# PRBonn/LiDiff

Hardware: NVIDIA H100
Metric: denoising_steps_per_sec_180k_pts_T50 (higher is better)
Workload: dtype fp16x3 split tensor-core MMA, fp32 accumulate (fp32 CUDA cores for the Cin=3 stem), fp64 DPM update

## Files before the change

### include/lidiff_b200.h

```cpp
#ifndef LIDIFF_B200_H_
#define LIDIFF_B200_H_

#include <stdint.h>
#include <stddef.h>

#ifdef __cplusplus
extern "C" {
#endif

#define LB2_OK            0
#define LB2_ERR_ARG      -1
#define LB2_ERR_CUDA     -2
#define LB2_ERR_UNSUP    -3

#define LB2_KEY_EMPTY 0xFFFFFFFFFFFFFFFFull

int         lb2_create(int device, void** handle);
void        lb2_destroy(void* handle);
const char* lb2_last_error(void* handle);
int         lb2_version(void);
int64_t     lb2_launch_count(void* handle);
int         lb2_read_status(void* handle, void* stream);

typedef struct {
    uint64_t* keys;
    int32_t*  vals;
    int32_t   cap_table;
} lb2_grid;

int lb2_quantize(void* h, void* stream, const float* x, int64_t n_elem, float resolution, int div_mode,
                 float* out_coord);

size_t lb2_unique_scratch_bytes(int64_t n_cap);
int lb2_unique_build(void* h, void* stream,
                     const float* in_f, const int32_t* in_i, const int32_t* d_nin, int32_t n_cap,
                     int32_t ts_floor, lb2_grid grid,
                     int32_t* out_coords, int32_t* inverse, int32_t* d_nout, void* scratch);

size_t lb2_voxel_mean_scratch_bytes(int32_t m_cap, int32_t c);
int lb2_voxel_mean(void* h, void* stream, const float* feats, const int32_t* inverse, int32_t n,
                   int32_t c, const int32_t* d_m, int32_t m_cap, float* out, void* scratch);

int lb2_kernel_map(void* h, void* stream, lb2_grid grid_in, const int32_t* out_coords,
                   const int32_t* d_nout, int32_t nout_cap, int32_t ks, int32_t step,
                   int32_t* nbr, int64_t nbr_stride, uint64_t* pair_count, uint32_t* row_mask);

int lb2_kernel_map_self(void* h, void* stream, lb2_grid grid, const int32_t* coords, const int32_t* d_n, int32_t n_cap,
                        int32_t step, int32_t* nbr, int64_t nbr_stride, uint64_t* pair_count, uint32_t* row_mask);

size_t lb2_row_order_scratch_bytes(int32_t n_cap);
int lb2_row_order(void* h, void* stream, const uint32_t* row_mask, const int32_t* d_n, int32_t n_cap,
                  int32_t kvol, int32_t* perm, void* scratch, const int32_t* coords, int32_t coord_shift);

int lb2_tile_order(void* h, void* stream, const uint32_t* row_mask, const int32_t* row_perm, const int32_t* d_n, int32_t n_cap,
                   int32_t* order128, int32_t* order256, void* scratch);

typedef struct {
    const float*   in1;
    const float*   in2;
    const float*   residual;
    float*         out;
    const float*   gate_table;
    const int32_t* gate_idx;
    float*         out_gated;
    const float*   pre_add;
    const void*    in1_h;
    const void*    in2_h;
    void*          out_h;
    void*          out_gated_h;
    const void*    residual_h;
} lb2_conv_io;

typedef struct {
    int32_t        c1, c2, cout, kvol;
    const float*   weight;
    const void*    weight_packed;
    const float*   scale;
    const float*   shift;
    int32_t        relu;
    const int32_t* nbr;
    int64_t        nbr_stride;
    const int32_t* d_mout;
    int32_t        mout_cap;
    const int32_t* row_perm;
    const uint32_t* row_mask;
    int32_t        npass;
    lb2_conv_io    io[2];
    const int32_t* tile_order128;
    const int32_t* tile_order256;
} lb2_conv_desc;

#define LB2_ALGO_AUTO  0
#define LB2_ALGO_FFMA  1
#define LB2_ALGO_TC    2
#define LB2_ALGO_TC_TILE 3
int lb2_spconv_forward(void* h, void* stream, const lb2_conv_desc* d, int algo);

typedef struct {
    int32_t        c1, c2, cout, kvol;
    const void*    weight_packed;
    const int32_t* pair_in;
    const int32_t* pair_out;
    const int32_t* koff;
    const int32_t* tile_off;
    int32_t        npass;
    const float*   in1[2];
    const float*   in2[2];
    const void*    in1_h[2];
    const void*    in2_h[2];
    float*         out[2];
    const int32_t* d_zero_rows;
    int32_t        zero_rows_cap;
} lb2_scatter_desc;
size_t lb2_pair_list_scratch_bytes(void);
int lb2_pair_list(void* h, void* stream, const int32_t* nbr, int64_t nbr_stride, const int32_t* d_nout,
                  int32_t nout_cap, int32_t kvol, int32_t skip_k, int32_t* pair_in, int32_t* pair_out,
                  int32_t* koff, int32_t* tile_off, void* scratch);
int lb2_spconv_scatter_supported(int32_t c1, int32_t c2, int32_t cout, int32_t kvol);
int lb2_spconv_scatter(void* h, void* stream, const lb2_scatter_desc* d);

size_t lb2_packed_weight_bytes(int32_t kvol, int32_t cin, int32_t cout);
int lb2_pack_weights(void* h, void* stream, const float* weight, int32_t kvol, int32_t cin, int32_t cout,
                     void* packed);

int lb2_nn_match(void* h, void* stream, const int32_t* q_coords, const int32_t* d_nq, int32_t nq_cap,
                 const int32_t* k_coords, const int32_t* d_nk, int32_t nk_cap, int32_t batch_scale,
                 int32_t* idx);

int lb2_nn_match_grid(void* h, void* stream, const int32_t* q_coords, const int32_t* d_nq, int32_t nq_cap,
                      const int32_t* k_coords, const int32_t* d_nk, int32_t nk_cap, lb2_grid key_grid,
                      int32_t key_stride, int32_t max_ring, int32_t* idx);

size_t lb2_nn_table_bytes(void);
int lb2_nn_table_build(void* h, void* stream, const int32_t* k_coords, const int32_t* d_nk, int32_t nk_cap, void* table);
int lb2_nn_match_table(void* h, void* stream, const int32_t* q_coords, const int32_t* d_nq, int32_t nq_cap,
                       const int32_t* k_coords, const int32_t* d_nk, int32_t nk_cap, const void* table,
                       int32_t key_stride, int32_t max_ring, int32_t* idx);

size_t lb2_nn_tree_bytes(int32_t nk_cap);
int lb2_nn_tree_build(void* h, void* stream, const int32_t* k_coords, const int32_t* d_nk, int32_t nk_cap, void* tree);
int lb2_nn_match_tree(void* h, void* stream, const int32_t* q_coords, const int32_t* d_nq, int32_t nq_cap,
                      const void* tree, int32_t nk_cap, const int32_t* k_coords, const int32_t* hint_of,
                      const int32_t* hint_idx, int32_t* idx);

int lb2_linear(void* h, void* stream, const float* x, int64_t ldx, const float* w, const float* b,
               const float* addend, int64_t ld_addend, int32_t m_cap, const int32_t* d_m,
               int32_t n_in, int32_t n_out, int32_t act, float* y, int64_t ldy,
               const float* prebias, int32_t pre_act);

int lb2_head_mlp(void* h, void* stream, const float* x, int64_t ldx, int64_t x_pass_stride, const float* w0, const float* b0,
                 const float* w1, const float* b1, int32_t m_cap, const int32_t* d_m, int32_t n_in, int32_t n_hid,
                 int32_t n_out, int32_t out_act, int32_t npass, float* y, int64_t ldy, int64_t y_pass_stride);

int lb2_gate_mul(void* h, void* stream, const float* x, const float* table, const int32_t* idx,
                 const int32_t* d_m, int32_t m_cap, int32_t c, float* out, void* out_h);

int lb2_gather_rows(void* h, void* stream, const float* src, const int32_t* idx, int32_t n, int32_t c,
                    float* out);

typedef struct {
    double c_sample, c_x0, c_noise, sigma_s, alpha_s, inv_r0;
    float  guidance_w, resolution;
    int32_t second_order, div_mode, f64_state;
} lb2_dpm_coef;
int lb2_guidance_dpm_step(void* h, void* stream, const float* eps_c, const float* eps_u,
                          const int32_t* inverse, const float* x_t, const double* x_init,
                          const float* noise, double* x0_state, int64_t n_points, lb2_dpm_coef coef,
                          float* eps_out, float* x_next, float* coord_next ,
                          const float* batch_col );

int lb2_farthest_point_sample(void* h, void* stream, const double* pts, int32_t n, int32_t n_samples,
                              int32_t* out_idx, double* dist_scratch);

int64_t lb2_fps_batched_capacity(void* h);
int lb2_farthest_point_sample_batched(void* h, void* stream, const double* pts, const int64_t* d_offsets, int32_t n_scans,
                                      int32_t max_n, int32_t n_samples, int32_t* out_idx);


size_t lb2_pc_tree_bytes(int32_t n_cap);
size_t lb2_pc_nn_scratch_bytes(int32_t nq_cap);
int lb2_pc_tree_build(void* h, void* stream, const double* pts, int32_t n, void* tree);
int lb2_pc_nn(void* h, void* stream, const double* q, int32_t nq, const void* tree, double* dist, int32_t* idx, void* scratch);

int lb2_pc_knn(void* h, void* stream, const void* tree, int32_t n, int32_t k, int32_t* idx, double* d2);
int lb2_pc_normals(void* h, void* stream, const double* pts, int32_t n, const int32_t* idx, int32_t k, double* normals);

int lb2_voxel_occupancy(void* h, void* stream, const double* pts, int32_t n, const double* edges, int32_t bins,
                        uint32_t* bits, uint32_t* counts, uint64_t* n_in);

int lb2_occupancy_confusion(void* h, void* stream, const uint32_t* bits_gt, const uint32_t* bits_pred, int64_t nbits, uint64_t* out);

int lb2_occupancy_bev(void* h, void* stream, const uint32_t* bits, int32_t bins, uint32_t* bev);

size_t lb2_jsd_scratch_bytes(int64_t n);
int lb2_jsd(void* h, void* stream, const uint32_t* hist_a, const uint32_t* hist_b, int64_t n, double* out, void* scratch);

size_t lb2_dist_stats_scratch_bytes(int32_t nt);
int lb2_dist_stats(void* h, void* stream, const double* dist, int32_t n, const double* thresholds, int32_t nt,
                   double* sum_out, uint64_t* counts_out, void* scratch);

#define LB2_MAP_AXIS_BITS 21
typedef struct { float m[12]; } lb2_pose;

int lb2_map_rehash(void* h, void* stream, lb2_grid old_table, lb2_grid table);

size_t lb2_map_scan_scratch_bytes(int32_t n_cap);
int lb2_map_scan(void* h, void* stream, const float* points, const uint32_t* labels, int32_t n, lb2_pose pose, float voxel_size,
                 int32_t div_mode, lb2_grid table, float* map, int32_t map_n, int32_t map_cap, int32_t* d_out, void* scratch);

#ifdef __cplusplus
}
#endif
#endif
```

### lidiff_b200/_lib.py

```python
from __future__ import annotations

import ctypes as C
import os
import threading

import torch

_SO = os.path.join(os.path.dirname(os.path.abspath(__file__)), "_C", "liblidiff_b200.so")

ALGO_AUTO, ALGO_FFMA, ALGO_TC, ALGO_TC_TILE = 0, 1, 2, 3


class Grid(C.Structure):
    _fields_ = [("keys", C.c_void_p), ("vals", C.c_void_p), ("cap_table", C.c_int32)]


class ConvIO(C.Structure):
    _fields_ = [("in1", C.c_void_p), ("in2", C.c_void_p), ("residual", C.c_void_p), ("out", C.c_void_p),
                ("gate_table", C.c_void_p), ("gate_idx", C.c_void_p), ("out_gated", C.c_void_p), ("pre_add", C.c_void_p),
                ("in1_h", C.c_void_p), ("in2_h", C.c_void_p), ("out_h", C.c_void_p), ("out_gated_h", C.c_void_p),
                ("residual_h", C.c_void_p)]


class ConvDesc(C.Structure):
    _fields_ = [("c1", C.c_int32), ("c2", C.c_int32), ("cout", C.c_int32), ("kvol", C.c_int32),
                ("weight", C.c_void_p), ("weight_packed", C.c_void_p),
                ("scale", C.c_void_p), ("shift", C.c_void_p), ("relu", C.c_int32),
                ("nbr", C.c_void_p), ("nbr_stride", C.c_int64),
                ("d_mout", C.c_void_p), ("mout_cap", C.c_int32), ("row_perm", C.c_void_p), ("row_mask", C.c_void_p),
                ("npass", C.c_int32),
                ("io", ConvIO * 2),
                ("tile_order128", C.c_void_p), ("tile_order256", C.c_void_p)]


class ScatterDesc(C.Structure):
    _fields_ = [("c1", C.c_int32), ("c2", C.c_int32), ("cout", C.c_int32), ("kvol", C.c_int32),
                ("weight_packed", C.c_void_p), ("pair_in", C.c_void_p), ("pair_out", C.c_void_p),
                ("koff", C.c_void_p), ("tile_off", C.c_void_p), ("npass", C.c_int32),
                ("in1", C.c_void_p * 2), ("in2", C.c_void_p * 2), ("in1_h", C.c_void_p * 2), ("in2_h", C.c_void_p * 2),
                ("out", C.c_void_p * 2),
                ("d_zero_rows", C.c_void_p), ("zero_rows_cap", C.c_int32)]


class DpmCoef(C.Structure):
    _fields_ = [("c_sample", C.c_double), ("c_x0", C.c_double), ("c_noise", C.c_double),
                ("sigma_s", C.c_double), ("alpha_s", C.c_double), ("inv_r0", C.c_double),
                ("guidance_w", C.c_float), ("resolution", C.c_float),
                ("second_order", C.c_int32), ("div_mode", C.c_int32), ("f64_state", C.c_int32)]


EXPORTS = [
    "lb2_create", "lb2_destroy", "lb2_last_error", "lb2_version", "lb2_launch_count", "lb2_read_status",
    "lb2_tile_order",
    "lb2_quantize", "lb2_unique_scratch_bytes", "lb2_unique_build", "lb2_voxel_mean_scratch_bytes", "lb2_voxel_mean", "lb2_kernel_map",
    "lb2_spconv_forward", "lb2_packed_weight_bytes", "lb2_pack_weights", "lb2_nn_match", "lb2_linear",
    "lb2_gate_mul", "lb2_gather_rows", "lb2_head_mlp", "lb2_kernel_map_self", "lb2_guidance_dpm_step", "lb2_farthest_point_sample",
    "lb2_row_order", "lb2_row_order_scratch_bytes", "lb2_nn_match_grid",
    "lb2_nn_table_bytes", "lb2_nn_table_build", "lb2_nn_match_table",
    "lb2_nn_tree_bytes", "lb2_nn_tree_build", "lb2_nn_match_tree",
    "lb2_pair_list", "lb2_pair_list_scratch_bytes", "lb2_spconv_scatter", "lb2_spconv_scatter_supported",
    "lb2_pc_tree_bytes", "lb2_pc_nn_scratch_bytes", "lb2_pc_tree_build", "lb2_pc_nn", "lb2_voxel_occupancy", "lb2_occupancy_confusion",
    "lb2_occupancy_bev", "lb2_jsd_scratch_bytes", "lb2_jsd", "lb2_dist_stats_scratch_bytes", "lb2_dist_stats",
    "lb2_map_rehash", "lb2_map_scan_scratch_bytes", "lb2_map_scan",
    "lb2_pc_knn", "lb2_pc_normals", "lb2_fps_batched_capacity", "lb2_farthest_point_sample_batched",
]


class Pose(C.Structure):
    _fields_ = [("m", C.c_float * 12)]


def _ptr(t):
    if t is None:
        return None
    if isinstance(t, int):
        return t
    return t.data_ptr()


class Lib:

    def __init__(self, path: str = _SO):
        if not os.path.exists(path):
            raise RuntimeError(f"lidiff_b200: CUDA library not built ({path}); run `python -c 'import __graft_entry__ as g; g.build()'` "
                               "or lidiff_b200/csrc/build.sh — there is no CPU fallback")
        self.path = path
        self.dll = C.CDLL(path)
        d = self.dll
        d.lb2_create.argtypes = [C.c_int, C.POINTER(C.c_void_p)]
        d.lb2_destroy.argtypes = [C.c_void_p]
        d.lb2_destroy.restype = None
        d.lb2_last_error.argtypes = [C.c_void_p]
        d.lb2_last_error.restype = C.c_char_p
        d.lb2_launch_count.argtypes = [C.c_void_p]
        d.lb2_launch_count.restype = C.c_int64
        d.lb2_read_status.argtypes = [C.c_void_p, C.c_void_p]
        d.lb2_unique_scratch_bytes.argtypes = [C.c_int64]
        d.lb2_unique_scratch_bytes.restype = C.c_size_t
        d.lb2_voxel_mean_scratch_bytes.argtypes = [C.c_int32, C.c_int32]
        d.lb2_voxel_mean_scratch_bytes.restype = C.c_size_t
        d.lb2_packed_weight_bytes.argtypes = [C.c_int32] * 3
        d.lb2_packed_weight_bytes.restype = C.c_size_t
        vp, i32, i64, f32 = C.c_void_p, C.c_int32, C.c_int64, C.c_float
        d.lb2_quantize.argtypes = [vp, vp, vp, i64, f32, C.c_int, vp]
        d.lb2_unique_build.argtypes = [vp, vp, vp, vp, vp, i32, i32, Grid, vp, vp, vp, vp]
        d.lb2_voxel_mean.argtypes = [vp, vp, vp, vp, i32, i32, vp, i32, vp, vp]
        d.lb2_kernel_map.argtypes = [vp, vp, Grid, vp, vp, i32, i32, i32, vp, i64, vp, vp]
        d.lb2_kernel_map_self.argtypes = [vp, vp, Grid, vp, vp, i32, i32, vp, i64, vp, vp]
        d.lb2_row_order.argtypes = [vp, vp, vp, vp, i32, i32, vp, vp, vp, i32]
        d.lb2_tile_order.argtypes = [vp, vp, vp, vp, vp, i32, vp, vp, vp]
        d.lb2_row_order_scratch_bytes.restype = C.c_size_t
        d.lb2_row_order_scratch_bytes.argtypes = [i32]
        d.lb2_spconv_forward.argtypes = [vp, vp, C.POINTER(ConvDesc), C.c_int]
        d.lb2_pack_weights.argtypes = [vp, vp, vp, i32, i32, i32, vp]
        d.lb2_nn_match.argtypes = [vp, vp, vp, vp, i32, vp, vp, i32, i32, vp]
        d.lb2_pair_list.argtypes = [vp, vp, vp, i64, vp, i32, i32, i32, vp, vp, vp, vp, vp]
        d.lb2_pair_list_scratch_bytes.restype = C.c_size_t
        d.lb2_spconv_scatter.argtypes = [vp, vp, C.POINTER(ScatterDesc)]
        d.lb2_spconv_scatter_supported.argtypes = [i32, i32, i32, i32]
        d.lb2_nn_table_bytes.restype = C.c_size_t
        d.lb2_nn_tree_bytes.restype = C.c_size_t
        d.lb2_nn_tree_bytes.argtypes = [i32]
        d.lb2_nn_tree_build.argtypes = [vp, vp, vp, vp, i32, vp]
        d.lb2_nn_match_tree.argtypes = [vp, vp, vp, vp, i32, vp, i32, vp, vp, vp, vp]
        d.lb2_nn_table_build.argtypes = [vp, vp, vp, vp, i32, vp]
        d.lb2_nn_match_table.argtypes = [vp, vp, vp, vp, i32, vp, vp, i32, vp, i32, i32, vp]
        d.lb2_nn_match_grid.argtypes = [vp, vp, vp, vp, i32, vp, vp, i32, Grid, i32, i32, vp]
        d.lb2_linear.argtypes = [vp, vp, vp, i64, vp, vp, vp, i64, i32, vp, i32, i32, i32, vp, i64,
                                 vp, i32]
        d.lb2_gate_mul.argtypes = [vp, vp, vp, vp, vp, vp, i32, i32, vp, vp]
        d.lb2_gather_rows.argtypes = [vp, vp, vp, vp, i32, i32, vp]
        d.lb2_head_mlp.argtypes = [vp, vp, vp, i64, i64, vp, vp, vp, vp, i32, vp, i32, i32, i32, i32, i32, vp, i64, i64]
        d.lb2_guidance_dpm_step.argtypes = [vp, vp, vp, vp, vp, vp, vp, vp, vp, i64, DpmCoef, vp, vp, vp, vp]
        d.lb2_farthest_point_sample.argtypes = [vp, vp, vp, i32, i32, vp, vp]
        d.lb2_fps_batched_capacity.argtypes = [vp]
        d.lb2_fps_batched_capacity.restype = C.c_int64
        d.lb2_farthest_point_sample_batched.argtypes = [vp, vp, vp, vp, i32, i32, i32, vp]
        for f, a in (("lb2_pc_tree_bytes", i32), ("lb2_pc_nn_scratch_bytes", i32), ("lb2_jsd_scratch_bytes", i64),
                     ("lb2_dist_stats_scratch_bytes", i32)):
            getattr(d, f).argtypes = [a]
            getattr(d, f).restype = C.c_size_t
        d.lb2_pc_tree_build.argtypes = [vp, vp, vp, i32, vp]
        d.lb2_pc_nn.argtypes = [vp, vp, vp, i32, vp, vp, vp, vp]
        d.lb2_pc_knn.argtypes = [vp, vp, vp, i32, i32, vp, vp]
        d.lb2_pc_normals.argtypes = [vp, vp, vp, i32, vp, i32, vp]
        d.lb2_voxel_occupancy.argtypes = [vp, vp, vp, i32, vp, i32, vp, vp, vp]
        d.lb2_occupancy_confusion.argtypes = [vp, vp, vp, vp, i64, vp]
        d.lb2_occupancy_bev.argtypes = [vp, vp, vp, i32, vp]
        d.lb2_jsd.argtypes = [vp, vp, vp, vp, i64, vp, vp]
        d.lb2_dist_stats.argtypes = [vp, vp, vp, i32, vp, i32, vp, vp, vp]
        d.lb2_map_rehash.argtypes = [vp, vp, Grid, Grid]
        d.lb2_map_scan_scratch_bytes.argtypes = [i32]
        d.lb2_map_scan_scratch_bytes.restype = C.c_size_t
        d.lb2_map_scan.argtypes = [vp, vp, vp, vp, i32, Pose, f32, i32, Grid, vp, i32, i32, vp, vp]
        self._handles = {}
        self._lock = threading.Lock()

    def missing_symbols(self):
        return [s for s in EXPORTS if not hasattr(self.dll, s)]

    def handle(self, device) -> "Handle":
        dev = torch.device(device)
        if dev.type != "cuda":
            raise RuntimeError("lidiff_b200 runs on CUDA (H100, sm_90a) only; no CPU fallback")
        idx = dev.index if dev.index is not None else torch.cuda.current_device()
        with self._lock:
            if idx not in self._handles:
                hp = C.c_void_p()
                rc = self.dll.lb2_create(idx, C.byref(hp))
                if rc != 0:
                    raise RuntimeError(f"lb2_create(device={idx}) failed with {rc} (needs an sm_90 GPU)")
                self._handles[idx] = Handle(self, hp, idx)
            return self._handles[idx]


class Handle:
    def __init__(self, lib: Lib, hp, device_index: int):
        self.lib, self.dll, self.hp, self.device_index = lib, lib.dll, hp, device_index
        self.device = torch.device("cuda", device_index)

    def _stream(self):
        return torch.cuda.current_stream(self.device).cuda_stream

    def _check(self, rc, what):
        if rc != 0:
            msg = self.dll.lb2_last_error(self.hp)
            raise RuntimeError(f"{what} failed ({rc}): {msg.decode() if msg else ''}")

    def launch_count(self) -> int:
        return int(self.dll.lb2_launch_count(self.hp))

    def read_status(self) -> int:
        return int(self.dll.lb2_read_status(self.hp, self._stream()))

    def new_grid(self, n_cap: int):
        cap = 1 << max(4, (2 * n_cap - 1).bit_length())
        keys = torch.empty(cap, dtype=torch.int64, device=self.device)
        vals = torch.empty(2 * cap, dtype=torch.int32, device=self.device)
        return (keys, vals, cap)

    @staticmethod
    def _grid(g):
        return Grid(g[0].data_ptr(), g[1].data_ptr(), g[2])

    def unique_scratch(self, n_cap: int) -> torch.Tensor:
        nbytes = int(self.dll.lb2_unique_scratch_bytes(n_cap))
        return torch.empty(nbytes, dtype=torch.uint8, device=self.device)

    def quantize(self, x, resolution, div_mode, out):
        self._check(self.dll.lb2_quantize(self.hp, self._stream(), _ptr(x), x.numel(), float(resolution), int(div_mode), _ptr(out)), "lb2_quantize")

    def unique_build(self, in_f, in_i, d_nin, n_cap, ts_floor, grid, out_coords, inverse, d_nout, scratch):
        self._check(self.dll.lb2_unique_build(self.hp, self._stream(), _ptr(in_f), _ptr(in_i), _ptr(d_nin), int(n_cap), int(ts_floor),
                                              self._grid(grid), _ptr(out_coords), _ptr(inverse), _ptr(d_nout), _ptr(scratch)), "lb2_unique_build")

    def voxel_mean_scratch(self, m_cap: int, c: int) -> torch.Tensor:
        nbytes = int(self.dll.lb2_voxel_mean_scratch_bytes(int(m_cap), int(c)))
        return torch.empty(nbytes, dtype=torch.uint8, device=self.device)

    def voxel_mean(self, feats, inverse, n, c, d_m, m_cap, out, scratch):
        self._check(self.dll.lb2_voxel_mean(self.hp, self._stream(), _ptr(feats), _ptr(inverse), int(n), int(c), _ptr(d_m), int(m_cap),
                                            _ptr(out), _ptr(scratch)), "lb2_voxel_mean")

    def kernel_map(self, grid_in, out_coords, d_nout, nout_cap, ks, step, nbr, nbr_stride, pair_count=None, row_mask=None):
        self._check(self.dll.lb2_kernel_map(self.hp, self._stream(), self._grid(grid_in), _ptr(out_coords), _ptr(d_nout), int(nout_cap),
                                            int(ks), int(step), _ptr(nbr), int(nbr_stride), _ptr(pair_count), _ptr(row_mask)), "lb2_kernel_map")

    def kernel_map_self(self, grid, coords, d_n, n_cap, step, nbr, nbr_stride, pair_count=None, row_mask=None):
        self._check(self.dll.lb2_kernel_map_self(self.hp, self._stream(), self._grid(grid), _ptr(coords), _ptr(d_n), int(n_cap), int(step),
                                                 _ptr(nbr), int(nbr_stride), _ptr(pair_count), _ptr(row_mask)), "lb2_kernel_map_self")

    def row_order_scratch_bytes(self, n_cap) -> int:
        return int(self.dll.lb2_row_order_scratch_bytes(int(n_cap)))

    def row_order(self, row_mask, d_n, n_cap, kvol, perm, scratch, coords=None, coord_shift=0):
        self._check(self.dll.lb2_row_order(self.hp, self._stream(), _ptr(row_mask), _ptr(d_n), int(n_cap), int(kvol), _ptr(perm), _ptr(scratch),
                                           _ptr(coords), int(coord_shift)), "lb2_row_order")

    def tile_order(self, row_mask, row_perm, d_n, n_cap, order128, order256, scratch):
        self._check(self.dll.lb2_tile_order(self.hp, self._stream(), _ptr(row_mask), _ptr(row_perm), _ptr(d_n), int(n_cap), _ptr(order128),
                                            _ptr(order256), _ptr(scratch)), "lb2_tile_order")

    def spconv(self, desc: ConvDesc, algo: int = ALGO_AUTO):
        self._check(self.dll.lb2_spconv_forward(self.hp, self._stream(), C.byref(desc), int(algo)), "lb2_spconv_forward")

    def pair_list(self, nbr, nbr_stride, d_nout, nout_cap, kvol, skip_k, pair_in, pair_out, koff, tile_off, scratch):
        self._check(self.dll.lb2_pair_list(self.hp, self._stream(), _ptr(nbr), int(nbr_stride), _ptr(d_nout), int(nout_cap), int(kvol), int(skip_k),
                                           _ptr(pair_in), _ptr(pair_out), _ptr(koff), _ptr(tile_off), _ptr(scratch)), "lb2_pair_list")

    def scatter_supported(self, c1, c2, cout, kvol) -> bool:
        return bool(self.dll.lb2_spconv_scatter_supported(int(c1), int(c2), int(cout), int(kvol)))

    def spconv_scatter(self, desc: "ScatterDesc"):
        self._check(self.dll.lb2_spconv_scatter(self.hp, self._stream(), C.byref(desc)), "lb2_spconv_scatter")

    def packed_weight_bytes(self, kvol, cin, cout) -> int:
        return int(self.dll.lb2_packed_weight_bytes(kvol, cin, cout))

    def pack_weights(self, w: torch.Tensor):
        kvol, cin, cout = w.shape
        nbytes = self.packed_weight_bytes(kvol, cin, cout)
        if nbytes == 0:
            return None
        out = torch.empty(nbytes, dtype=torch.uint8, device=self.device)
        self._check(self.dll.lb2_pack_weights(self.hp, self._stream(), _ptr(w), kvol, cin, cout, _ptr(out)), "lb2_pack_weights")
        return out

    def nn_match(self, q, d_nq, nq_cap, k, d_nk, nk_cap, batch_scale, idx):
        self._check(self.dll.lb2_nn_match(self.hp, self._stream(), _ptr(q), _ptr(d_nq), int(nq_cap), _ptr(k), _ptr(d_nk), int(nk_cap),
                                          int(batch_scale), _ptr(idx)), "lb2_nn_match")

    def nn_match_grid(self, q, d_nq, nq_cap, k, d_nk, nk_cap, key_grid, key_stride, max_ring, idx):
        self._check(self.dll.lb2_nn_match_grid(self.hp, self._stream(), _ptr(q), _ptr(d_nq), int(nq_cap), _ptr(k), _ptr(d_nk), int(nk_cap),
                                               self._grid(key_grid), int(key_stride), int(max_ring), _ptr(idx)), "lb2_nn_match_grid")

    def nn_table(self, k, d_nk, nk_cap):
        t = torch.empty(int(self.dll.lb2_nn_table_bytes()), dtype=torch.uint8, device=self.device)
        self._check(self.dll.lb2_nn_table_build(self.hp, self._stream(), _ptr(k), _ptr(d_nk), int(nk_cap), _ptr(t)), "lb2_nn_table_build")
        return t

    def nn_tree(self, k, d_nk, nk_cap, out=None):
        nbytes = int(self.dll.lb2_nn_tree_bytes(int(nk_cap)))
        t = out if (out is not None and out.numel() == nbytes) else torch.empty(nbytes, dtype=torch.uint8, device=self.device)
        self._check(self.dll.lb2_nn_tree_build(self.hp, self._stream(), _ptr(k), _ptr(d_nk), int(nk_cap), _ptr(t)), "lb2_nn_tree_build")
        return t

    def nn_match_tree(self, q, d_nq, nq_cap, tree, nk_cap, idx, k=None, hint_of=None, hint_idx=None):
        self._check(self.dll.lb2_nn_match_tree(self.hp, self._stream(), _ptr(q), _ptr(d_nq), int(nq_cap), _ptr(tree), int(nk_cap),
                                               _ptr(k), _ptr(hint_of), _ptr(hint_idx), _ptr(idx)), "lb2_nn_match_tree")

    def nn_match_table(self, q, d_nq, nq_cap, k, d_nk, nk_cap, table, key_stride, max_ring, idx):
        self._check(self.dll.lb2_nn_match_table(self.hp, self._stream(), _ptr(q), _ptr(d_nq), int(nq_cap), _ptr(k), _ptr(d_nk), int(nk_cap),
                                                _ptr(table), int(key_stride), int(max_ring), _ptr(idx)), "lb2_nn_match_table")

    def linear(self, x, ldx, w, b, addend, ld_add, m_cap, d_m, n_in, n_out, act, y, ldy, prebias=None, pre_act=0):
        self._check(self.dll.lb2_linear(self.hp, self._stream(), _ptr(x), int(ldx), _ptr(w), _ptr(b), _ptr(addend), int(ld_add), int(m_cap),
                                        _ptr(d_m), int(n_in), int(n_out), int(act), _ptr(y), int(ldy), _ptr(prebias), int(pre_act)), "lb2_linear")

    def head_mlp(self, x, ldx, x_pass_stride, w0, b0, w1, b1, m_cap, d_m, n_in, n_hid, n_out, out_act, npass, y, ldy, y_pass_stride):
        self._check(self.dll.lb2_head_mlp(self.hp, self._stream(), _ptr(x), int(ldx), int(x_pass_stride), _ptr(w0), _ptr(b0), _ptr(w1), _ptr(b1),
                                          int(m_cap), _ptr(d_m), int(n_in), int(n_hid), int(n_out), int(out_act), int(npass), _ptr(y), int(ldy),
                                          int(y_pass_stride)), "lb2_head_mlp")

    def gate_mul(self, x, table, idx, d_m, m_cap, c, out, out_h=None):
        self._check(self.dll.lb2_gate_mul(self.hp, self._stream(), _ptr(x), _ptr(table), _ptr(idx), _ptr(d_m), int(m_cap), int(c), _ptr(out),
                                          _ptr(out_h)), "lb2_gate_mul")

    def gather_rows(self, src, idx, n, c, out):
        self._check(self.dll.lb2_gather_rows(self.hp, self._stream(), _ptr(src), _ptr(idx), int(n), int(c), _ptr(out)), "lb2_gather_rows")

    def guidance_dpm_step(self, eps_c, eps_u, inverse, x_t, x_init, noise, x0_state, n_points, coef: DpmCoef,
                          eps_out, x_next, coord_next, batch_col=None):
        self._check(self.dll.lb2_guidance_dpm_step(self.hp, self._stream(), _ptr(eps_c), _ptr(eps_u), _ptr(inverse), _ptr(x_t), _ptr(x_init),
                                                   _ptr(noise), _ptr(x0_state), int(n_points), coef, _ptr(eps_out), _ptr(x_next),
                                                   _ptr(coord_next), _ptr(batch_col)), "lb2_guidance_dpm_step")

    def farthest_point_sample(self, pts, n, n_samples, out_idx, dist):
        self._check(self.dll.lb2_farthest_point_sample(self.hp, self._stream(), _ptr(pts), int(n), int(n_samples), _ptr(out_idx), _ptr(dist)),
                    "lb2_farthest_point_sample")

    def fps_batched_capacity(self) -> int:
        return int(self.dll.lb2_fps_batched_capacity(self.hp))

    def farthest_point_sample_batched(self, pts, offsets, n_scans, max_n, n_samples, out_idx):
        self._check(self.dll.lb2_farthest_point_sample_batched(self.hp, self._stream(), _ptr(pts), _ptr(offsets), int(n_scans), int(max_n),
                                                               int(n_samples), _ptr(out_idx)), "lb2_farthest_point_sample_batched")

    def _bytes(self, nbytes):
        return torch.empty(max(int(nbytes), 1), dtype=torch.uint8, device=self.device)

    def pc_tree(self, pts):
        n = pts.shape[0]
        tree = self._bytes(self.dll.lb2_pc_tree_bytes(n))
        self._check(self.dll.lb2_pc_tree_build(self.hp, self._stream(), _ptr(pts), int(n), _ptr(tree)), "lb2_pc_tree_build")
        return tree

    def pc_nn(self, q, tree, dist, idx=None):
        nq = q.shape[0]
        scratch = self._bytes(self.dll.lb2_pc_nn_scratch_bytes(nq))
        self._check(self.dll.lb2_pc_nn(self.hp, self._stream(), _ptr(q), int(nq), _ptr(tree), _ptr(dist), _ptr(idx), _ptr(scratch)),
                    "lb2_pc_nn")

    def pc_knn(self, tree, n, k, idx, d2=None):
        self._check(self.dll.lb2_pc_knn(self.hp, self._stream(), _ptr(tree), int(n), int(k), _ptr(idx), _ptr(d2)), "lb2_pc_knn")

    def pc_normals(self, pts, idx, normals):
        n, k = idx.shape
        self._check(self.dll.lb2_pc_normals(self.hp, self._stream(), _ptr(pts), int(n), _ptr(idx), int(k), _ptr(normals)), "lb2_pc_normals")

    def voxel_occupancy(self, pts, edges, bits=None, counts=None, n_in=None):
        bins = edges.shape[0] - 1
        self._check(self.dll.lb2_voxel_occupancy(self.hp, self._stream(), _ptr(pts), int(pts.shape[0]), _ptr(edges), int(bins), _ptr(bits),
                                                 _ptr(counts), _ptr(n_in)), "lb2_voxel_occupancy")

    def occupancy_confusion(self, bits_gt, bits_pred, nbits, out):
        self._check(self.dll.lb2_occupancy_confusion(self.hp, self._stream(), _ptr(bits_gt), _ptr(bits_pred), int(nbits), _ptr(out)),
                    "lb2_occupancy_confusion")

    def occupancy_bev(self, bits, bins, bev):
        self._check(self.dll.lb2_occupancy_bev(self.hp, self._stream(), _ptr(bits), int(bins), _ptr(bev)), "lb2_occupancy_bev")

    def jsd(self, hist_a, hist_b, out):
        n = hist_a.numel()
        scratch = self._bytes(self.dll.lb2_jsd_scratch_bytes(n))
        self._check(self.dll.lb2_jsd(self.hp, self._stream(), _ptr(hist_a), _ptr(hist_b), int(n), _ptr(out), _ptr(scratch)), "lb2_jsd")

    def dist_stats(self, dist, thresholds, sum_out, counts_out):
        nt = thresholds.shape[0]
        scratch = self._bytes(self.dll.lb2_dist_stats_scratch_bytes(nt))
        self._check(self.dll.lb2_dist_stats(self.hp, self._stream(), _ptr(dist), int(dist.shape[0]), _ptr(thresholds), int(nt), _ptr(sum_out),
                                            _ptr(counts_out), _ptr(scratch)), "lb2_dist_stats")

    def new_map_table(self, cap: int):
        return (torch.empty(cap, dtype=torch.int64, device=self.device), torch.empty(2 * cap, dtype=torch.int32, device=self.device), cap)

    def map_rehash(self, old, table):
        self._check(self.dll.lb2_map_rehash(self.hp, self._stream(), self._grid(old) if old is not None else Grid(None, None, 0),
                                            self._grid(table)), "lb2_map_rehash")

    def map_scan_scratch(self, n_cap: int) -> torch.Tensor:
        return self._bytes(self.dll.lb2_map_scan_scratch_bytes(int(n_cap)))

    def map_scan(self, points, labels, pose12, voxel_size, div_mode, table, map_buf, map_n, out, scratch):
        pose = Pose((C.c_float * 12)(*[float(v) for v in pose12]))
        self._check(self.dll.lb2_map_scan(self.hp, self._stream(), _ptr(points), _ptr(labels), int(points.shape[0]), pose, float(voxel_size),
                                          int(div_mode), self._grid(table), _ptr(map_buf), int(map_n), int(map_buf.shape[0]), _ptr(out),
                                          _ptr(scratch)), "lb2_map_scan")


_LIB = None


def get_lib() -> Lib:
    global _LIB
    if _LIB is None:
        _LIB = Lib()
    return _LIB


def get_handle(device) -> Handle:
    return get_lib().handle(device)
```

### lidiff_b200/csrc/api.cu

```cuda
#include "common.cuh"

int lb2_spconv_ffma_launch(Lb2Handle* h, cudaStream_t s, const lb2_conv_desc* d);
int lb2_spconv_tc_launch(Lb2Handle* h, cudaStream_t s, const lb2_conv_desc* d);
bool lb2_spconv_tc_supported(const lb2_conv_desc* d);

extern "C" int lb2_spconv_forward(void* handle, void* stream, const lb2_conv_desc* d, int algo) {
    Lb2Handle* h = (Lb2Handle*)handle;
    LB2_REQUIRE(h, h && d, "spconv_forward null");
    LB2_REQUIRE(h, d->npass == 1 || d->npass == 2, "npass must be 1 or 2");
    LB2_REQUIRE(h, d->c1 > 0 && d->c2 >= 0 && d->cout > 0 && d->kvol > 0 && d->mout_cap > 0, "shape");
    LB2_REQUIRE(h, d->weight != nullptr, "weight");
    LB2_REQUIRE(h, (d->scale == nullptr) == (d->shift == nullptr), "scale/shift must come together");
    LB2_REQUIRE(h, d->nbr != nullptr || d->kvol == 1, "identity map only for kvol == 1");
    LB2_REQUIRE(h, d->nbr == nullptr || d->nbr_stride >= d->mout_cap, "nbr_stride");
    bool have_f32 = true;
    for (int p = 0; p < d->npass; ++p) {
        const lb2_conv_io& io = d->io[p];
        const bool f = io.in1 && (d->c2 == 0 || io.in2), hh = io.in1_h && (d->c2 == 0 || io.in2_h);
        LB2_REQUIRE(h, f || hh, "in1 / in2 (fp32 tensors or their split companions)");
        LB2_REQUIRE(h, d->c2 > 0 || (io.in2 == nullptr && io.in2_h == nullptr), "in2 / c2 mismatch");
        LB2_REQUIRE(h, !hh || (d->c1 % 8 == 0 && d->c2 % 8 == 0), "split companions need channel counts that are multiples of 8");
        LB2_REQUIRE(h, io.out || io.out_gated || io.out_h || io.out_gated_h, "no output");
        have_f32 = have_f32 && f;
    }
    LB2_REQUIRE(h, d->c2 == 0 || d->c1 % 16 == 0, "c1 must be a multiple of 16 when in2 is given");
    cudaStream_t s = (cudaStream_t)stream;
    if (algo == LB2_ALGO_TC || algo == LB2_ALGO_TC_TILE) {
        if (!d->weight_packed || !lb2_spconv_tc_supported(d))
            return lb2_fail(h, LB2_ERR_UNSUP, "tensor-core variant does not support this layer%s", "");
        return lb2_spconv_tc_launch(h, s, d);
    }
    if (algo == LB2_ALGO_AUTO && d->weight_packed && lb2_spconv_tc_supported(d)) return lb2_spconv_tc_launch(h, s, d);
    if (!have_f32) return lb2_fail(h, LB2_ERR_UNSUP, "companion-only inputs need a tensor-core variant that takes this layer%s", "");
    return lb2_spconv_ffma_launch(h, s, d);
}
```

### lidiff_b200/csrc/coords.cu

```cuda
#include "common.cuh"
#include <stdlib.h>
#include <limits.h>
#include <algorithm>

extern "C" int lb2_version(void) { return 100; }

extern "C" int lb2_create(int device, void** handle) {
    if (!handle) return LB2_ERR_ARG;
    *handle = nullptr;
    int n = 0;
    if (cudaGetDeviceCount(&n) != cudaSuccess || n <= 0 || device < 0 || device >= n) return LB2_ERR_CUDA;
    if (cudaSetDevice(device) != cudaSuccess) return LB2_ERR_CUDA;
    cudaDeviceProp prop;
    if (cudaGetDeviceProperties(&prop, device) != cudaSuccess) return LB2_ERR_CUDA;
    if (prop.major != 9) return LB2_ERR_UNSUP;
    Lb2Handle* h = new Lb2Handle();
    h->device = device; h->num_sms = prop.multiProcessorCount; h->launches = 0; h->err[0] = 0; h->configured = 0;
    if (cudaMalloc(&h->d_status, sizeof(int32_t)) != cudaSuccess) { delete h; return LB2_ERR_CUDA; }
    cudaMemset(h->d_status, 0, sizeof(int32_t));
    *handle = h;
    return LB2_OK;
}

extern "C" void lb2_destroy(void* handle) {
    Lb2Handle* h = (Lb2Handle*)handle;
    if (!h) return;
    cudaFree(h->d_status);
    delete h;
}

extern "C" const char* lb2_last_error(void* handle) {
    return handle ? ((Lb2Handle*)handle)->err : "null handle";
}

extern "C" int64_t lb2_launch_count(void* handle) { return handle ? ((Lb2Handle*)handle)->launches : -1; }

extern "C" int lb2_read_status(void* handle, void* stream) {
    Lb2Handle* h = (Lb2Handle*)handle;
    if (!h) return LB2_ERR_ARG;
    int32_t v = 0;
    cudaStream_t s = (cudaStream_t)stream;
    if (cudaMemcpyAsync(&v, h->d_status, sizeof(v), cudaMemcpyDeviceToHost, s) != cudaSuccess) return LB2_ERR_CUDA;
    if (cudaMemsetAsync(h->d_status, 0, sizeof(v), s) != cudaSuccess) return LB2_ERR_CUDA;
    if (cudaStreamSynchronize(s) != cudaSuccess) return LB2_ERR_CUDA;
    return v;
}

__global__ void k_quantize(const float* __restrict__ x, long long n, float res, float inv_res, int div_mode,
                           float* __restrict__ out) {
    long long i = (long long)blockIdx.x * blockDim.x + threadIdx.x;
    if (i >= n) return;
    float v = x[i];
    float q = div_mode == 0 ? __fdiv_rn(v, res) : __fmul_rn(v, inv_res);
    out[i] = rintf(q);
}

extern "C" int lb2_quantize(void* handle, void* stream, const float* x, int64_t n_elem, float resolution,
                            int div_mode, float* out_coord) {
    Lb2Handle* h = (Lb2Handle*)handle;
    LB2_REQUIRE(h, h && x && out_coord && resolution > 0.f, "quantize");
    if (n_elem == 0) return LB2_OK;
    float inv = 1.0f / resolution;
    k_quantize<<<cdiv(n_elem, 256), 256, 0, (cudaStream_t)stream>>>(x, n_elem, resolution, inv, div_mode, out_coord);
    LB2_POST_LAUNCH(h, "k_quantize");
    return LB2_OK;
}

#define SCAN_THREADS 512
#define SCAN_ITEMS   4
#define SCAN_TILE    (SCAN_THREADS * SCAN_ITEMS)

struct UniqueScratch {
    int* slot_of;
    int* rank;
    int* bsum;
};

extern "C" size_t lb2_unique_scratch_bytes(int64_t n_cap) {
    size_t a = ((size_t)n_cap * sizeof(int) + 255) / 256 * 256;
    return 2 * a + SCAN_TILE * sizeof(int) + 256;
}

static UniqueScratch carve(void* scratch, int64_t n_cap) {
    size_t a = ((size_t)n_cap * sizeof(int) + 255) / 256 * 256;
    char* p = (char*)scratch;
    UniqueScratch s;
    s.slot_of = (int*)p; s.rank = (int*)(p + a); s.bsum = (int*)(p + 2 * a);
    return s;
}

__global__ void k_grid_clear(unsigned long long* keys, int* vals, int cap) {
    int i = blockIdx.x * blockDim.x + threadIdx.x;
    if (i < cap) { keys[i] = LB2_KEY_EMPTY; vals[i] = INT_MAX; vals[cap + i] = -1; }
}

__device__ __forceinline__ int4 load_row(const float* __restrict__ in_f, const int* __restrict__ in_i, int i, int ts, bool* nan = nullptr) {
    int4 c;
    if (in_f) {
        float4 f = __ldg(reinterpret_cast<const float4*>(in_f) + i);
        c = make_int4((int)floorf(f.x), (int)floorf(f.y), (int)floorf(f.z), (int)floorf(f.w));
        if (nan) *nan = isnan(f.x) || isnan(f.y) || isnan(f.z) || isnan(f.w);
    } else {
        c = __ldg(reinterpret_cast<const int4*>(in_i) + i);
    }
    if (ts > 0) { c.y = floor_to_multiple(c.y, ts); c.z = floor_to_multiple(c.z, ts); c.w = floor_to_multiple(c.w, ts); }
    return c;
}

__global__ void k_grid_insert(const float* __restrict__ in_f, const int* __restrict__ in_i,
                              const int* __restrict__ d_n, int n_cap, int ts,
                              unsigned long long* keys, int* vals, unsigned mask,
                              int* __restrict__ slot_of, int* status) {
    int i = blockIdx.x * blockDim.x + threadIdx.x;
    int n = d_n ? min(*d_n, n_cap) : n_cap;
    if (i >= n) return;
    bool nan = false;
    int4 c = load_row(in_f, in_i, i, ts, &nan);
    unsigned long long key;
    if (!lb2_pack_key(c.x, c.y, c.z, c.w, key) || nan) atomicOr(status, 1);
    unsigned slot = lb2_hash(key) & mask;
    while (true) {
        unsigned long long prev = atomicCAS(keys + slot, (unsigned long long)LB2_KEY_EMPTY, key);
        if (prev == LB2_KEY_EMPTY || prev == key) break;
        slot = (slot + 1) & mask;
    }
    atomicMin(vals + slot, i);
    slot_of[i] = (int)slot;
}

__global__ void __launch_bounds__(SCAN_THREADS) k_scan_local(const int* __restrict__ slot_of, const int* __restrict__ vals,
                                                             const int* __restrict__ d_n, int n_cap,
                                                             int* __restrict__ rank, int* __restrict__ bsum) {
    __shared__ int warp_tot[SCAN_THREADS / 32];
    int n = d_n ? min(*d_n, n_cap) : n_cap;
    int base = blockIdx.x * SCAN_TILE + threadIdx.x * SCAN_ITEMS;
    int f[SCAN_ITEMS], tsum = 0;
#pragma unroll
    for (int j = 0; j < SCAN_ITEMS; ++j) {
        int i = base + j;
        f[j] = (i < n) ? (vals[slot_of[i]] == i) : 0;
        tsum += f[j];
    }
    int lane = threadIdx.x & 31, w = threadIdx.x >> 5;
    int incl = tsum;
#pragma unroll
    for (int d = 1; d < 32; d <<= 1) { int v = __shfl_up_sync(0xffffffffu, incl, d); if (lane >= d) incl += v; }
    if (lane == 31) warp_tot[w] = incl;
    __syncthreads();
    if (w == 0) {
        int v = (lane < SCAN_THREADS / 32) ? warp_tot[lane] : 0, inc2 = v;
#pragma unroll
        for (int d = 1; d < 32; d <<= 1) { int u = __shfl_up_sync(0xffffffffu, inc2, d); if (lane >= d) inc2 += u; }
        if (lane < SCAN_THREADS / 32) warp_tot[lane] = inc2 - v;
        if (lane == SCAN_THREADS / 32 - 1) bsum[blockIdx.x] = inc2;
    }
    __syncthreads();
    int excl = warp_tot[w] + incl - tsum;
#pragma unroll
    for (int j = 0; j < SCAN_ITEMS; ++j) {
        int i = base + j;
        if (i < n) rank[i] = f[j] ? excl : -1;
        excl += f[j];
    }
}

__global__ void __launch_bounds__(SCAN_THREADS) k_scan_bsum(int* __restrict__ bsum, int nblocks, int* __restrict__ d_total) {
    __shared__ int warp_tot[SCAN_THREADS / 32];
    int base = threadIdx.x * SCAN_ITEMS;
    int v[SCAN_ITEMS], tsum = 0;
#pragma unroll
    for (int j = 0; j < SCAN_ITEMS; ++j) { v[j] = (base + j < nblocks) ? bsum[base + j] : 0; tsum += v[j]; }
    int lane = threadIdx.x & 31, w = threadIdx.x >> 5;
    int incl = tsum;
#pragma unroll
    for (int d = 1; d < 32; d <<= 1) { int u = __shfl_up_sync(0xffffffffu, incl, d); if (lane >= d) incl += u; }
    if (lane == 31) warp_tot[w] = incl;
    __syncthreads();
    if (w == 0) {
        int x = (lane < SCAN_THREADS / 32) ? warp_tot[lane] : 0, inc2 = x;
#pragma unroll
        for (int d = 1; d < 32; d <<= 1) { int u = __shfl_up_sync(0xffffffffu, inc2, d); if (lane >= d) inc2 += u; }
        if (lane < SCAN_THREADS / 32) warp_tot[lane] = inc2 - x;
        if (lane == SCAN_THREADS / 32 - 1) *d_total = inc2;
    }
    __syncthreads();
    int excl = warp_tot[w] + incl - tsum;
#pragma unroll
    for (int j = 0; j < SCAN_ITEMS; ++j) { if (base + j < nblocks) bsum[base + j] = excl; excl += v[j]; }
}

__global__ void k_unique_emit(const float* __restrict__ in_f, const int* __restrict__ in_i,
                              const int* __restrict__ d_n, int n_cap, int ts,
                              const int* __restrict__ slot_of, const int* __restrict__ rank,
                              const int* __restrict__ bsum, int* __restrict__ vals, int cap,
                              int4* __restrict__ out_coords) {
    int i = blockIdx.x * blockDim.x + threadIdx.x;
    int n = d_n ? min(*d_n, n_cap) : n_cap;
    if (i >= n) return;
    int r = rank[i];
    if (r < 0) return;
    r += bsum[i / SCAN_TILE];
    vals[cap + slot_of[i]] = r;
    out_coords[r] = load_row(in_f, in_i, i, ts);
}

__global__ void k_unique_inverse(const int* __restrict__ d_n, int n_cap, const int* __restrict__ slot_of,
                                 const int* __restrict__ vals, int cap, int* __restrict__ inverse) {
    int i = blockIdx.x * blockDim.x + threadIdx.x;
    int n = d_n ? min(*d_n, n_cap) : n_cap;
    if (i < n) inverse[i] = vals[cap + slot_of[i]];
}

extern "C" int lb2_unique_build(void* handle, void* stream, const float* in_f, const int32_t* in_i,
                                const int32_t* d_nin, int32_t n_cap, int32_t ts_floor, lb2_grid grid,
                                int32_t* out_coords, int32_t* inverse, int32_t* d_nout, void* scratch) {
    Lb2Handle* h = (Lb2Handle*)handle;
    LB2_REQUIRE(h, h != nullptr, "handle");
    LB2_REQUIRE(h, (in_f != nullptr) != (in_i != nullptr), "exactly one of in_f / in_i");
    LB2_REQUIRE(h, grid.keys && grid.vals && out_coords && d_nout && scratch, "null buffer");
    LB2_REQUIRE(h, n_cap > 0 && n_cap <= SCAN_TILE * SCAN_TILE, "n_cap out of range (max 4M rows)");
    LB2_REQUIRE(h, grid.cap_table >= 2 && (grid.cap_table & (grid.cap_table - 1)) == 0, "cap_table must be a power of two");
    LB2_REQUIRE(h, (long long)grid.cap_table >= 2LL * n_cap, "cap_table must be >= 2 * n_cap");
    LB2_REQUIRE(h, ts_floor >= 0, "ts_floor");
    cudaStream_t s = (cudaStream_t)stream;
    UniqueScratch sc = carve(scratch, n_cap);
    unsigned long long* keys = (unsigned long long*)grid.keys;
    int cap = grid.cap_table;
    unsigned mask = (unsigned)cap - 1u;
    int nblk = (int)cdiv(n_cap, SCAN_TILE);

    k_grid_clear<<<cdiv(cap, 256), 256, 0, s>>>(keys, grid.vals, cap);
    LB2_POST_LAUNCH(h, "k_grid_clear");
    k_grid_insert<<<cdiv(n_cap, 256), 256, 0, s>>>(in_f, in_i, d_nin, n_cap, ts_floor, keys, grid.vals, mask, sc.slot_of, h->d_status);
    LB2_POST_LAUNCH(h, "k_grid_insert");
    k_scan_local<<<nblk, SCAN_THREADS, 0, s>>>(sc.slot_of, grid.vals, d_nin, n_cap, sc.rank, sc.bsum);
    LB2_POST_LAUNCH(h, "k_scan_local");
    k_scan_bsum<<<1, SCAN_THREADS, 0, s>>>(sc.bsum, nblk, d_nout);
    LB2_POST_LAUNCH(h, "k_scan_bsum");
    k_unique_emit<<<cdiv(n_cap, 256), 256, 0, s>>>(in_f, in_i, d_nin, n_cap, ts_floor, sc.slot_of, sc.rank, sc.bsum,
                                                  grid.vals, cap, (int4*)out_coords);
    LB2_POST_LAUNCH(h, "k_unique_emit");
    if (inverse) {
        k_unique_inverse<<<cdiv(n_cap, 256), 256, 0, s>>>(d_nin, n_cap, sc.slot_of, grid.vals, cap, inverse);
        LB2_POST_LAUNCH(h, "k_unique_inverse");
    }
    return LB2_OK;
}

__device__ __forceinline__ int voxel_fix_shift(float maxabs, int count) {
    int e;
    frexpf(maxabs, &e);
    return 61 - e - (32 - __clz(count));
}

__global__ void k_voxel_absmax(const float* __restrict__ feats, const int* __restrict__ inverse, int n, int c,
                               unsigned* __restrict__ maxabs, int* __restrict__ counts) {
    long long t = (long long)blockIdx.x * blockDim.x + threadIdx.x;
    if (t >= (long long)n * c) return;
    int i = (int)(t / c), j = (int)(t % c);
    int r = inverse[i];
    atomicMax(maxabs + (long long)r * c + j, __float_as_uint(fabsf(feats[t])));
    if (j == 0) atomicAdd(counts + r, 1);
}

__global__ void k_voxel_accum(const float* __restrict__ feats, const int* __restrict__ inverse, int n, int c,
                              const float* __restrict__ maxabs, const int* __restrict__ counts, unsigned long long* __restrict__ sums) {
    long long t = (long long)blockIdx.x * blockDim.x + threadIdx.x;
    if (t >= (long long)n * c) return;
    int i = (int)(t / c), j = (int)(t % c);
    int r = inverse[i];
    const long long e = (long long)r * c + j;
    const float m = maxabs[e];
    if (!(m > 0.f) || !isfinite(m)) return;
    const long long q = llrint(ldexp((double)feats[t], voxel_fix_shift(m, counts[r])));
    atomicAdd(sums + e, (unsigned long long)q);
}

__global__ void k_voxel_div(float* __restrict__ out, const int* __restrict__ counts, const unsigned long long* __restrict__ sums,
                            const int* __restrict__ d_m, int m_cap, int c) {
    long long t = (long long)blockIdx.x * blockDim.x + threadIdx.x;
    int m = d_m ? min(*d_m, m_cap) : m_cap;
    if (t >= (long long)m * c) return;
    const float mx = out[t];
    const int cnt = counts[t / c];
    if (!isfinite(mx)) { out[t] = __int_as_float(0x7fffffff); return; }
    if (!(mx > 0.f) || cnt == 0) { out[t] = cnt == 0 ? __fdiv_rn(0.f, 0.f) : 0.f; return; }
    const double sum = ldexp((double)(long long)sums[t], -voxel_fix_shift(mx, cnt));
    out[t] = __double2float_rn(sum / (double)cnt);
}

extern "C" size_t lb2_voxel_mean_scratch_bytes(int32_t m_cap, int32_t c) {
    return (size_t)m_cap * c * sizeof(unsigned long long) + (size_t)m_cap * sizeof(int);
}

extern "C" int lb2_voxel_mean(void* handle, void* stream, const float* feats, const int32_t* inverse, int32_t n,
                              int32_t c, const int32_t* d_m, int32_t m_cap, float* out, void* scratch) {
    Lb2Handle* h = (Lb2Handle*)handle;
    LB2_REQUIRE(h, h && feats && inverse && out && scratch && n > 0 && c > 0 && m_cap > 0, "voxel_mean");
    cudaStream_t s = (cudaStream_t)stream;
    unsigned long long* sums = (unsigned long long*)scratch;
    int* counts = (int*)(sums + (size_t)m_cap * c);
    if (cudaMemsetAsync(out, 0, (size_t)m_cap * c * sizeof(float), s) != cudaSuccess ||
        cudaMemsetAsync(scratch, 0, lb2_voxel_mean_scratch_bytes(m_cap, c), s) != cudaSuccess)
        return lb2_fail(h, LB2_ERR_CUDA, "voxel_mean memset%s", "");
    k_voxel_absmax<<<cdiv((long long)n * c, 256), 256, 0, s>>>(feats, inverse, n, c, (unsigned*)out, counts);
    LB2_POST_LAUNCH(h, "k_voxel_absmax");
    k_voxel_accum<<<cdiv((long long)n * c, 256), 256, 0, s>>>(feats, inverse, n, c, out, counts, sums);
    LB2_POST_LAUNCH(h, "k_voxel_accum");
    k_voxel_div<<<cdiv((long long)m_cap * c, 256), 256, 0, s>>>(out, counts, sums, d_m, m_cap, c);
    LB2_POST_LAUNCH(h, "k_voxel_div");
    return LB2_OK;
}

template <int KS>
__global__ void __launch_bounds__(128) k_kernel_map(const unsigned long long* __restrict__ keys, const int* __restrict__ rows, unsigned mask,
                                                    const int4* __restrict__ out_coords, const int* __restrict__ d_n, int n_cap,
                                                    int step, int* __restrict__ nbr, long long nbr_stride,
                                                    unsigned long long* __restrict__ pair_count, unsigned* __restrict__ row_mask) {
    constexpr int KV = KS * KS * KS;
    const int o = blockIdx.x * blockDim.x + threadIdx.x;
    const int n = d_n ? min(*d_n, n_cap) : n_cap;
    unsigned found = 0;
    if (o < n) {
        const int4 c = __ldg(out_coords + o);
        constexpr int cen = (KS & 1) ? KS / 2 : 0;
        int res[KV];
        unsigned long long key[KV], got[KV];
        unsigned slot[KV];
#pragma unroll
        for (int k = 0; k < KV; ++k) {
            const int kx = k % KS, ky = (k / KS) % KS, kz = k / (KS * KS);
            const int x = c.y + (kx - cen) * step, y = c.z + (ky - cen) * step, z = c.w + (kz - cen) * step;
            const bool ok = lb2_pack_key(c.x, x, y, z, key[k]);
            slot[k] = ok ? (lb2_hash(key[k]) & mask) : 0u;
            got[k] = ok ? __ldg(keys + slot[k]) : LB2_KEY_EMPTY;
            if (!ok) key[k] = ~LB2_KEY_EMPTY;
        }
#pragma unroll
        for (int k = 0; k < KV; ++k) {
            if (got[k] == key[k]) res[k] = __ldg(rows + slot[k]);
            else if (got[k] == LB2_KEY_EMPTY) res[k] = -1;
            else {
                unsigned sl = (slot[k] + 1) & mask;
                res[k] = -1;
                while (true) {
                    const unsigned long long kk = __ldg(keys + sl);
                    if (kk == key[k]) { res[k] = __ldg(rows + sl); break; }
                    if (kk == LB2_KEY_EMPTY) break;
                    sl = (sl + 1) & mask;
                }
            }
        }
#pragma unroll
        for (int k = 0; k < KV; ++k) {
            nbr[(long long)k * nbr_stride + o] = res[k];
            if (res[k] >= 0) found |= 1u << k;
        }
    } else if (o < n_cap) {
#pragma unroll
        for (int k = 0; k < KV; ++k) nbr[(long long)k * nbr_stride + o] = -1;
    }
    if (row_mask && o < n_cap) row_mask[o] = found;
    if (pair_count) {
        int cnt = __popc(found);
#pragma unroll
        for (int d = 16; d > 0; d >>= 1) cnt += __shfl_xor_sync(0xffffffffu, cnt, d);
        if ((threadIdx.x & 31) == 0 && cnt) atomicAdd(pair_count, (unsigned long long)cnt);
    }
}

extern "C" int lb2_kernel_map(void* handle, void* stream, lb2_grid grid_in, const int32_t* out_coords,
                              const int32_t* d_nout, int32_t nout_cap, int32_t ks, int32_t step,
                              int32_t* nbr, int64_t nbr_stride, uint64_t* pair_count, uint32_t* row_mask) {
    Lb2Handle* h = (Lb2Handle*)handle;
    LB2_REQUIRE(h, h && grid_in.keys && grid_in.vals && out_coords && nbr, "kernel_map null");
    LB2_REQUIRE(h, ks >= 1 && ks <= 3 && step != 0 && nout_cap > 0 && nbr_stride >= nout_cap, "kernel_map args");
    const unsigned long long* gk = (const unsigned long long*)grid_in.keys;
    const int* gr = grid_in.vals + grid_in.cap_table;
    const unsigned gm = (unsigned)grid_in.cap_table - 1u;
    const unsigned blocks = cdiv(nout_cap, 128);
    cudaStream_t s = (cudaStream_t)stream;
    if (ks == 3) k_kernel_map<3><<<blocks, 128, 0, s>>>(gk, gr, gm, (const int4*)out_coords, d_nout, nout_cap, step, nbr, nbr_stride, (unsigned long long*)pair_count, row_mask);
    else if (ks == 2) k_kernel_map<2><<<blocks, 128, 0, s>>>(gk, gr, gm, (const int4*)out_coords, d_nout, nout_cap, step, nbr, nbr_stride, (unsigned long long*)pair_count, row_mask);
    else k_kernel_map<1><<<blocks, 128, 0, s>>>(gk, gr, gm, (const int4*)out_coords, d_nout, nout_cap, step, nbr, nbr_stride, (unsigned long long*)pair_count, row_mask);
    LB2_POST_LAUNCH(h, "k_kernel_map");
    return LB2_OK;
}

__global__ void __launch_bounds__(128) k_kernel_map_self(const unsigned long long* __restrict__ keys, const int* __restrict__ rows, unsigned mask,
                                                         const int4* __restrict__ coords, const int* __restrict__ d_n, int n_cap, int step,
                                                         int* __restrict__ nbr, long long nbr_stride,
                                                         unsigned long long* __restrict__ pair_count, unsigned* __restrict__ row_mask) {
    constexpr int HALF = 13;
    const int o = blockIdx.x * blockDim.x + threadIdx.x;
    const int n = d_n ? min(*d_n, n_cap) : n_cap;
    unsigned found = 0;
    if (o < n) {
        const int4 c = __ldg(coords + o);
        int res[HALF];
        unsigned long long key[HALF], got[HALF];
        unsigned slot[HALF];
#pragma unroll
        for (int k = 0; k < HALF; ++k) {
            const int kx = k % 3, ky = (k / 3) % 3, kz = k / 9;
            const int x = c.y + (kx - 1) * step, y = c.z + (ky - 1) * step, z = c.w + (kz - 1) * step;
            const bool ok = lb2_pack_key(c.x, x, y, z, key[k]);
            slot[k] = ok ? (lb2_hash(key[k]) & mask) : 0u;
            got[k] = ok ? __ldg(keys + slot[k]) : LB2_KEY_EMPTY;
            if (!ok) key[k] = ~LB2_KEY_EMPTY;
        }
#pragma unroll
        for (int k = 0; k < HALF; ++k) {
            if (got[k] == key[k]) res[k] = __ldg(rows + slot[k]);
            else if (got[k] == LB2_KEY_EMPTY) res[k] = -1;
            else {
                unsigned sl = (slot[k] + 1) & mask;
                res[k] = -1;
                while (true) {
                    const unsigned long long kk = __ldg(keys + sl);
                    if (kk == key[k]) { res[k] = __ldg(rows + sl); break; }
                    if (kk == LB2_KEY_EMPTY) break;
                    sl = (sl + 1) & mask;
                }
            }
        }
#pragma unroll
        for (int k = 0; k < HALF; ++k) {
            nbr[(long long)k * nbr_stride + o] = res[k];
            if (res[k] >= 0) {
                found |= 1u << k;
                nbr[(long long)(26 - k) * nbr_stride + res[k]] = o;
                if (row_mask) atomicOr(row_mask + res[k], 1u << (26 - k));
            }
        }
        nbr[(long long)HALF * nbr_stride + o] = o;
        if (row_mask) atomicOr(row_mask + o, found | (1u << HALF));
    } else if (o < n_cap) {
#pragma unroll
        for (int k = 0; k <= HALF; ++k) nbr[(long long)k * nbr_stride + o] = -1;
    }
    if (pair_count) {
        int cnt = (o < n) ? 2 * __popc(found) + 1 : 0;
#pragma unroll
        for (int d = 16; d > 0; d >>= 1) cnt += __shfl_xor_sync(0xffffffffu, cnt, d);
        if ((threadIdx.x & 31) == 0 && cnt) atomicAdd(pair_count, (unsigned long long)cnt);
    }
}

extern "C" int lb2_kernel_map_self(void* handle, void* stream, lb2_grid grid, const int32_t* coords, const int32_t* d_n, int32_t n_cap,
                                   int32_t step, int32_t* nbr, int64_t nbr_stride, uint64_t* pair_count, uint32_t* row_mask) {
    Lb2Handle* h = (Lb2Handle*)handle;
    LB2_REQUIRE(h, h && grid.keys && grid.vals && coords && nbr, "kernel_map_self null");
    LB2_REQUIRE(h, step > 0 && n_cap > 0 && nbr_stride >= n_cap, "kernel_map_self args");
    cudaStream_t s = (cudaStream_t)stream;
    cudaError_t e = cudaMemsetAsync(nbr + 14 * nbr_stride, 0xff, (size_t)13 * nbr_stride * sizeof(int32_t), s);
    if (e == cudaSuccess && row_mask) e = cudaMemsetAsync(row_mask, 0, (size_t)n_cap * sizeof(uint32_t), s);
    if (e != cudaSuccess) return lb2_fail(h, LB2_ERR_CUDA, "kernel_map_self memset: %s", cudaGetErrorString(e));
    k_kernel_map_self<<<cdiv(n_cap, 128), 128, 0, s>>>((const unsigned long long*)grid.keys, grid.vals + grid.cap_table, (unsigned)grid.cap_table - 1u,
                                                       (const int4*)coords, d_n, n_cap, step, nbr, nbr_stride, (unsigned long long*)pair_count, row_mask);
    LB2_POST_LAUNCH(h, "k_kernel_map_self");
    return LB2_OK;
}

#define RS_BITS 9
#define RS_BINS (1 << RS_BITS)
#define RS_CHUNK 2048
#define RS_WARPS 8

__device__ __forceinline__ unsigned ro_key27(unsigned mask) {
    const unsigned extras = mask & ~(1u << 13);
    const unsigned k26 = ((mask >> 14) << 13) | (mask & 0x1fffu);
    return ((__popc(extras) >= 2) ? (1u << 26) : 0u) | k26;
}

__device__ __forceinline__ unsigned ro_part9(unsigned v) {
    v &= 0x1ffu;
    v = (v | (v << 16)) & 0x030000ffu;
    v = (v | (v << 8)) & 0x0300f00fu;
    v = (v | (v << 4)) & 0x030c30c3u;
    v = (v | (v << 2)) & 0x09249249u;
    return v;
}
__device__ __forceinline__ unsigned ro_morton(const int4 c, int shift) {
    return ro_part9((unsigned)(c.y >> shift)) | (ro_part9((unsigned)(c.z >> shift)) << 1) | (ro_part9((unsigned)(c.w >> shift)) << 2);
}

struct RsSrc {
    const unsigned* keys;
    const unsigned* mask;
    const int4* coords;
    const int* vals;
    int mode, coord_shift;
};
__device__ __forceinline__ unsigned rs_key(const RsSrc& s, int i) {
    switch (s.mode) {
        case 0: return s.keys[i];
        case 1: return ro_key27(s.mask[i]);
        case 2: return ro_morton(s.coords[i], s.coord_shift);
        case 4: return s.mask[i] & 0xffu;
        default: return ro_key27(s.mask[s.vals[i]]);
    }
}

__global__ void __launch_bounds__(256) k_rs_hist(const RsSrc src, const int* __restrict__ d_n, int n_cap, int shift, int* __restrict__ hist,
                                                 int* __restrict__ total) {
    __shared__ int sh[RS_BINS];
    for (int i = threadIdx.x; i < RS_BINS; i += blockDim.x) sh[i] = 0;
    __syncthreads();
    const int n = d_n ? min(*d_n, n_cap) : n_cap;
    const int lo = blockIdx.x * RS_CHUNK, hi = min(lo + RS_CHUNK, n);
    for (int i = lo + threadIdx.x; i < hi; i += blockDim.x) atomicAdd(&sh[(rs_key(src, i) >> shift) & (RS_BINS - 1)], 1);
    __syncthreads();
    for (int i = threadIdx.x; i < RS_BINS; i += blockDim.x) {
        hist[blockIdx.x * RS_BINS + i] = sh[i];
        if (sh[i]) atomicAdd(total + i, sh[i]);
    }
}

__global__ void __launch_bounds__(32 * RS_WARPS) k_rs_scatter(const RsSrc src, const int* __restrict__ d_n, int n_cap,
                                                              int shift, const int* __restrict__ hist, const int* __restrict__ total,
                                                              unsigned* __restrict__ keys_out, int* __restrict__ vals_out) {
    const int* __restrict__ vals_in = src.vals;
    __shared__ int cnt[RS_WARPS][RS_BINS];
    __shared__ int first[RS_BINS];
    const int warp = threadIdx.x >> 5, lane = threadIdx.x & 31;
    for (int i = threadIdx.x; i < RS_WARPS * RS_BINS; i += blockDim.x) (&cnt[0][0])[i] = 0;
    {
        const int t = threadIdx.x;
        const int t0 = total[2 * t], t1 = total[2 * t + 1];
        first[t] = t0 + t1;
        __syncthreads();
        for (int d = 1; d < RS_BINS / 2; d <<= 1) {
            const int u = (t >= d) ? first[t - d] : 0;
            __syncthreads();
            first[t] += u;
            __syncthreads();
        }
        const int excl = first[t] - (t0 + t1);
        int p0 = 0, p1 = 0;
#pragma unroll 8
        for (int b = 0; b < (int)blockIdx.x; ++b) {
            const int2 v = *reinterpret_cast<const int2*>(hist + b * RS_BINS + 2 * t);
            p0 += v.x; p1 += v.y;
        }
        __syncthreads();
        first[2 * t] = excl + p0;
        first[2 * t + 1] = excl + t0 + p1;
    }
    __syncthreads();
    const int n = d_n ? min(*d_n, n_cap) : n_cap;
    const int w0 = blockIdx.x * RS_CHUNK + warp * (RS_CHUNK / RS_WARPS);
    for (int g = 0; g < RS_CHUNK / RS_WARPS / 32; ++g) {
        const int i = w0 + g * 32 + lane;
        if (i < n) atomicAdd(&cnt[warp][(rs_key(src, i) >> shift) & (RS_BINS - 1)], 1);
    }
    __syncthreads();
    for (int bin = threadIdx.x; bin < RS_BINS; bin += blockDim.x) {
        int run = first[bin];
        for (int w = 0; w < RS_WARPS; ++w) { const int v = cnt[w][bin]; cnt[w][bin] = run; run += v; }
    }
    __syncthreads();
    for (int g = 0; g < RS_CHUNK / RS_WARPS / 32; ++g) {
        const int i = w0 + g * 32 + lane;
        const bool ok = i < n;
        const unsigned active = __ballot_sync(0xffffffffu, ok);
        if (ok) {
            const unsigned key = rs_key(src, i);
            const int val = vals_in ? vals_in[i] : i;
            const int d = (key >> shift) & (RS_BINS - 1);
            const unsigned peers = __match_any_sync(active, d);
            const int rank = __popc(peers & ((1u << lane) - 1u));
            const int pos = cnt[warp][d] + rank;
            __syncwarp(active);
            if (rank == 0) cnt[warp][d] += __popc(peers);
            __syncwarp(active);
            if (keys_out) keys_out[pos] = key;
            vals_out[pos] = val;
        }
    }
}

static int rs_blocks(int n_cap) { return cdiv(n_cap, RS_CHUNK); }

extern "C" size_t lb2_row_order_scratch_bytes(int32_t n_cap) {
    return ((size_t)RS_BINS * (rs_blocks(n_cap) + 6) + 3 * (size_t)n_cap) * sizeof(int);
}

extern "C" int lb2_row_order(void* handle, void* stream, const uint32_t* row_mask, const int32_t* d_n, int32_t n_cap,
                             int32_t kvol, int32_t* perm, void* scratch, const int32_t* coords, int32_t coord_shift) {
    Lb2Handle* h = (Lb2Handle*)handle;
    LB2_REQUIRE(h, h && row_mask && perm && scratch && n_cap > 0 && (kvol == 27 || (kvol >= 1 && kvol <= 8)), "row_order");
    LB2_REQUIRE(h, coord_shift >= 0 && coord_shift < 24, "row_order coord_shift");
    cudaStream_t s = (cudaStream_t)stream;
    if (kvol == 27) {
        const int nblk = rs_blocks(n_cap);
        int* hist = (int*)scratch;
        int* total = hist + (size_t)RS_BINS * nblk;
        unsigned* keys_a = (unsigned*)(total + 6 * RS_BINS);
        if (cudaMemsetAsync(total, 0, 6 * RS_BINS * sizeof(int), s) != cudaSuccess) return lb2_fail(h, LB2_ERR_CUDA, "row_order memset%s", "");
        unsigned* keys_b = keys_a + n_cap;
        int* vals_a = (int*)(keys_b + n_cap);
        const int npass = coords ? 6 : 3;
        for (int pass = 0; pass < npass; ++pass) {
            const int mp = coords ? pass - 3 : pass;
            const bool to_perm = coords ? (pass & 1) : !(pass & 1);
            RsSrc src;
            src.mask = row_mask; src.coords = (const int4*)coords; src.coord_shift = coord_shift;
            src.keys = (pass & 1) ? keys_a : keys_b;
            src.vals = (pass == 0) ? nullptr : (to_perm ? vals_a : perm);
            src.mode = (pass == 0) ? (coords ? 2 : 1) : ((coords && pass == 3) ? 3 : 0);
            unsigned* kout = (pass == npass - 1 || (coords && pass == 2)) ? nullptr : ((pass & 1) ? keys_b : keys_a);
            int* vout = to_perm ? perm : vals_a;
            const int shift = (mp >= 0 ? mp : pass) * RS_BITS;
            k_rs_hist<<<nblk, 256, 0, s>>>(src, d_n, n_cap, shift, hist, total + pass * RS_BINS);
            LB2_POST_LAUNCH(h, "k_rs_hist");
            k_rs_scatter<<<nblk, 32 * RS_WARPS, 0, s>>>(src, d_n, n_cap, shift, hist, total + pass * RS_BINS, kout, vout);
            LB2_POST_LAUNCH(h, "k_rs_scatter");
        }
        return LB2_OK;
    }
    const int nblk = rs_blocks(n_cap);
    int* hist = (int*)scratch;
    int* total = hist + (size_t)RS_BINS * nblk;
    if (cudaMemsetAsync(total, 0, RS_BINS * sizeof(int), s) != cudaSuccess) return lb2_fail(h, LB2_ERR_CUDA, "row_order memset%s", "");
    RsSrc src;
    src.mask = row_mask; src.coords = nullptr; src.coord_shift = 0; src.keys = nullptr; src.vals = nullptr; src.mode = 4;
    k_rs_hist<<<nblk, 256, 0, s>>>(src, d_n, n_cap, 0, hist, total);
    LB2_POST_LAUNCH(h, "k_rs_hist");
    k_rs_scatter<<<nblk, 32 * RS_WARPS, 0, s>>>(src, d_n, n_cap, 0, hist, total, nullptr, perm);
    LB2_POST_LAUNCH(h, "k_rs_scatter");
    return LB2_OK;
}

size_t rs_sort_scratch_bytes(int n_cap, int nbits) {
    return ((size_t)RS_BINS * (rs_blocks(n_cap) + cdiv(nbits, RS_BITS)) + 4 * (size_t)n_cap) * sizeof(int);
}

int rs_sort_keys(Lb2Handle* h, cudaStream_t s, const unsigned* keys, const int* d_n, int n_cap, int nbits, int* order, void* scratch) {
    const int nblk = rs_blocks(n_cap), npass = (int)cdiv(nbits, RS_BITS);
    int* hist = (int*)scratch;
    int* total = hist + (size_t)RS_BINS * nblk;
    unsigned* keys_a = (unsigned*)(total + (size_t)npass * RS_BINS);
    unsigned* keys_b = keys_a + n_cap;
    int* vals_a = (int*)(keys_b + n_cap);
    int* vals_b = vals_a + n_cap;
    if (cudaMemsetAsync(total, 0, (size_t)npass * RS_BINS * sizeof(int), s) != cudaSuccess) return lb2_fail(h, LB2_ERR_CUDA, "rs_sort memset%s", "");
    const unsigned* kin = keys;
    const int* vin = nullptr;
    for (int pass = 0; pass < npass; ++pass) {
        const bool last = pass == npass - 1;
        unsigned* kout = last ? nullptr : ((pass & 1) ? keys_b : keys_a);
        int* vout = last ? order : ((pass & 1) ? vals_b : vals_a);
        RsSrc src;
        src.keys = kin; src.mask = nullptr; src.coords = nullptr; src.vals = vin; src.mode = 0; src.coord_shift = 0;
        k_rs_hist<<<nblk, 256, 0, s>>>(src, d_n, n_cap, pass * RS_BITS, hist, total + pass * RS_BINS);
        LB2_POST_LAUNCH(h, "k_rs_hist");
        k_rs_scatter<<<nblk, 32 * RS_WARPS, 0, s>>>(src, d_n, n_cap, pass * RS_BITS, hist, total + pass * RS_BINS, kout, vout);
        LB2_POST_LAUNCH(h, "k_rs_scatter");
        kin = kout; vin = vout;
    }
    return LB2_OK;
}

#define NT_LEAF 4
#define NT_HDR 16

static int nt_nleaf(int nk_cap) { int n = 1; while (n * NT_LEAF < nk_cap) n <<= 1; return n; }
static size_t nt_sort_ints(int nk_cap) { return (size_t)RS_BINS * (rs_blocks(nk_cap) + 3) + 4 * (size_t)nk_cap; }

extern "C" size_t lb2_nn_tree_bytes(int32_t nk_cap) {
    return (NT_HDR + (size_t)2 * nt_nleaf(nk_cap) * 8 + 5 * (size_t)nt_nleaf(nk_cap) * NT_LEAF + nt_sort_ints(nk_cap)) * sizeof(int) + 64;
}

__global__ void k_nt_init(int* __restrict__ hdr, int nleaf, int nk_cap) {
    if (threadIdx.x < 3) { hdr[threadIdx.x] = 0x7fffffff; hdr[3 + threadIdx.x] = (int)0x80000000; }
    if (threadIdx.x == 0) { hdr[6] = 0; hdr[7] = nleaf; hdr[8] = nk_cap; }
}

__global__ void k_nt_minmax(const int4* __restrict__ keys, const int* __restrict__ d_nk, int nk_cap, int* __restrict__ hdr) {
    const int nk = d_nk ? min(*d_nk, nk_cap) : nk_cap;
    int lo[3] = {0x7fffffff, 0x7fffffff, 0x7fffffff}, hi[3] = {(int)0x80000000, (int)0x80000000, (int)0x80000000};
    for (int i = blockIdx.x * blockDim.x + threadIdx.x; i < nk; i += gridDim.x * blockDim.x) {
        const int4 c = __ldg(keys + i);
        lo[0] = min(lo[0], c.y); lo[1] = min(lo[1], c.z); lo[2] = min(lo[2], c.w);
        hi[0] = max(hi[0], c.y); hi[1] = max(hi[1], c.z); hi[2] = max(hi[2], c.w);
    }
#pragma unroll
    for (int a = 0; a < 3; ++a) {
#pragma unroll
        for (int o = 16; o > 0; o >>= 1) { lo[a] = min(lo[a], __shfl_xor_sync(0xffffffffu, lo[a], o)); hi[a] = max(hi[a], __shfl_xor_sync(0xffffffffu, hi[a], o)); }
        if ((threadIdx.x & 31) == 0) { atomicMin(hdr + a, lo[a]); atomicMax(hdr + 3 + a, hi[a]); }
    }
}

__device__ __forceinline__ unsigned nt_spread9(unsigned v) {
    unsigned r = 0;
#pragma unroll
    for (int b = 0; b < 9; ++b) r |= ((v >> b) & 1u) << (3 * b);
    return r;
}

__global__ void k_nt_morton(const int4* __restrict__ keys, const int* __restrict__ d_nk, int nk_cap, const int* __restrict__ hdr,
                            unsigned* __restrict__ codes) {
    const int nk = d_nk ? min(*d_nk, nk_cap) : nk_cap;
    const int i = blockIdx.x * blockDim.x + threadIdx.x;
    if (i >= nk) return;
    long long ext = 0;
#pragma unroll
    for (int a = 0; a < 3; ++a) ext = max(ext, (long long)hdr[3 + a] - (long long)hdr[a]);
    int shift = 0;
    while ((ext >> shift) > 511) ++shift;
    const int4 c = __ldg(keys + i);
    const unsigned x = (unsigned)(((long long)c.y - hdr[0]) >> shift), y = (unsigned)(((long long)c.z - hdr[1]) >> shift),
                   z = (unsigned)(((long long)c.w - hdr[2]) >> shift);
    codes[i] = nt_spread9(x) | (nt_spread9(y) << 1) | (nt_spread9(z) << 2);
}

__global__ void k_nt_gather(const int4* __restrict__ keys, const int* __restrict__ d_nk, int nk_cap, const int* __restrict__ order,
                            int slots, int4* __restrict__ skeys, int* __restrict__ sbatch) {
    const int nk = d_nk ? min(*d_nk, nk_cap) : nk_cap;
    const int i = blockIdx.x * blockDim.x + threadIdx.x;
    if (i >= slots) return;
    if (i >= nk) { skeys[i] = make_int4(0, 0, 0, -1); sbatch[i] = 0; return; }
    const int j = order[i];
    const int4 c = __ldg(keys + j);
    skeys[i] = make_int4(c.y, c.z, c.w, j);
    sbatch[i] = c.x;
}

__global__ void k_nt_leaves(const int4* __restrict__ skeys, const int* __restrict__ sbatch, const int* __restrict__ d_nk, int nk_cap,
                            int nleaf, int* __restrict__ nodes) {
    const int nk = d_nk ? min(*d_nk, nk_cap) : nk_cap;
    const int l = blockIdx.x * blockDim.x + threadIdx.x;
    if (l >= nleaf) return;
    int v[8] = {0x7fffffff, 0x7fffffff, 0x7fffffff, (int)0x80000000, (int)0x80000000, (int)0x80000000, 0x7fffffff, (int)0x80000000};
    for (int t = 0; t < NT_LEAF; ++t) {
        const int i = l * NT_LEAF + t;
        if (i >= nk) break;
        const int4 c = skeys[i];
        const int b = sbatch[i];
        v[0] = min(v[0], c.x); v[1] = min(v[1], c.y); v[2] = min(v[2], c.z);
        v[3] = max(v[3], c.x); v[4] = max(v[4], c.y); v[5] = max(v[5], c.z);
        v[6] = min(v[6], b); v[7] = max(v[7], b);
    }
    int* n = nodes + (size_t)(nleaf + l) * 8;
#pragma unroll
    for (int a = 0; a < 8; ++a) n[a] = v[a];
}

__global__ void __launch_bounds__(1024) k_nt_internal(int nleaf, int* __restrict__ nodes) {
    for (int first = nleaf >> 1; first >= 1; first >>= 1) {
        for (int i = first + threadIdx.x; i < 2 * first; i += blockDim.x) {
            const int* a = nodes + (size_t)(2 * i) * 8;
            const int* b = a + 8;
            int* n = nodes + (size_t)i * 8;
#pragma unroll
            for (int c = 0; c < 3; ++c) { n[c] = min(a[c], b[c]); n[3 + c] = max(a[3 + c], b[3 + c]); }
            n[6] = min(a[6], b[6]); n[7] = max(a[7], b[7]);
        }
        __syncthreads();
    }
}

extern "C" int lb2_nn_tree_build(void* handle, void* stream, const int32_t* k_coords, const int32_t* d_nk, int32_t nk_cap, void* tree) {
    Lb2Handle* h = (Lb2Handle*)handle;
    LB2_REQUIRE(h, h && k_coords && tree && nk_cap > 0, "nn_tree_build");
    cudaStream_t s = (cudaStream_t)stream;
    const int nleaf = nt_nleaf(nk_cap);
    int* hdr = (int*)tree;
    int* nodes = hdr + NT_HDR;
    int4* skeys = (int4*)(nodes + (size_t)2 * nleaf * 8);
    const int slots = nleaf * NT_LEAF;
    int* sbatch = (int*)(skeys + slots);
    int* hist = sbatch + slots;
    const int nblk = rs_blocks(nk_cap);
    int* total = hist + (size_t)RS_BINS * nblk;
    unsigned* codes = (unsigned*)(total + 3 * RS_BINS);
    unsigned* keys_b = codes + nk_cap;
    int* vals_a = (int*)(keys_b + nk_cap);
    int* vals_b = vals_a + nk_cap;
    k_nt_init<<<1, 32, 0, s>>>(hdr, nleaf, nk_cap);
    LB2_POST_LAUNCH(h, "k_nt_init");
    k_nt_minmax<<<std::min<unsigned>(cdiv(nk_cap, 256), 256u), 256, 0, s>>>((const int4*)k_coords, d_nk, nk_cap, hdr);
    LB2_POST_LAUNCH(h, "k_nt_minmax");
    k_nt_morton<<<cdiv(nk_cap, 256), 256, 0, s>>>((const int4*)k_coords, d_nk, nk_cap, hdr, codes);
    LB2_POST_LAUNCH(h, "k_nt_morton");
    if (cudaMemsetAsync(total, 0, 3 * RS_BINS * sizeof(int), s) != cudaSuccess) return lb2_fail(h, LB2_ERR_CUDA, "nn_tree memset%s", "");
    const unsigned* kin[3] = {codes, keys_b, codes};
    const int* vin[3] = {nullptr, vals_a, vals_b};
    unsigned* kout[3] = {keys_b, codes, nullptr};
    int* vout[3] = {vals_a, vals_b, vals_a};
    for (int pass = 0; pass < 3; ++pass) {
        RsSrc src;
        src.keys = kin[pass]; src.mask = nullptr; src.coords = nullptr; src.vals = vin[pass]; src.mode = 0; src.coord_shift = 0;
        k_rs_hist<<<nblk, 256, 0, s>>>(src, d_nk, nk_cap, pass * RS_BITS, hist, total + pass * RS_BINS);
        LB2_POST_LAUNCH(h, "k_rs_hist");
        k_rs_scatter<<<nblk, 32 * RS_WARPS, 0, s>>>(src, d_nk, nk_cap, pass * RS_BITS, hist, total + pass * RS_BINS, kout[pass], vout[pass]);
        LB2_POST_LAUNCH(h, "k_rs_scatter");
    }
    k_nt_gather<<<cdiv(slots, 256), 256, 0, s>>>((const int4*)k_coords, d_nk, nk_cap, vals_a, slots, skeys, sbatch);
    LB2_POST_LAUNCH(h, "k_nt_gather");
    k_nt_leaves<<<cdiv(nleaf, 256), 256, 0, s>>>(skeys, sbatch, d_nk, nk_cap, nleaf, nodes);
    LB2_POST_LAUNCH(h, "k_nt_leaves");
    k_nt_internal<<<1, 1024, 0, s>>>(nleaf, nodes);
    LB2_POST_LAUNCH(h, "k_nt_internal");
    return LB2_OK;
}

__global__ void __launch_bounds__(256) k_tile_masks(const unsigned* __restrict__ mask, const int* __restrict__ perm, const int* __restrict__ d_n,
                                                    int n_cap, unsigned* __restrict__ tmask) {
    const int n = d_n ? min(*d_n, n_cap) : n_cap;
    const int nt = (n + 127) >> 7;
    const int warp = (blockIdx.x * blockDim.x + threadIdx.x) >> 5, lane = threadIdx.x & 31;
    if (warp >= nt) return;
    unsigned m = 0;
#pragma unroll
    for (int q = 0; q < 4; ++q) {
        const int slot = warp * 128 + q * 32 + lane;
        if (slot < n) m |= __ldg(mask + (perm ? __ldg(perm + slot) : slot));
    }
    m = __reduce_or_sync(0xffffffffu, m);
    if (lane == 0) tmask[warp] = m;
}

__global__ void __launch_bounds__(1024) k_tile_sort(const unsigned* __restrict__ tmask, const int* __restrict__ d_n, int n_cap,
                                                    int* __restrict__ order128, int* __restrict__ order256) {
    __shared__ int bins[2][33];
    const int n = d_n ? min(*d_n, n_cap) : n_cap;
    const int nt128 = (n + 127) >> 7, nt256 = (n + 255) >> 8;
    const int cap128 = (n_cap + 127) >> 7, cap256 = (n_cap + 255) >> 8;
    if (threadIdx.x < 66) (&bins[0][0])[threadIdx.x] = 0;
    __syncthreads();
    for (int t = threadIdx.x; t < nt128; t += blockDim.x) atomicAdd(&bins[0][32 - __popc(tmask[t])], 1);
    for (int u = threadIdx.x; u < nt256; u += blockDim.x) {
        const unsigned m = tmask[2 * u] | ((2 * u + 1 < nt128) ? tmask[2 * u + 1] : 0u);
        atomicAdd(&bins[1][32 - __popc(m)], 1);
    }
    __syncthreads();
    if (threadIdx.x < 2) {
        int run = 0;
        for (int b = 0; b < 33; ++b) { const int v = bins[threadIdx.x][b]; bins[threadIdx.x][b] = run; run += v; }
    }
    __syncthreads();
    for (int t = threadIdx.x; t < nt128; t += blockDim.x) order128[atomicAdd(&bins[0][32 - __popc(tmask[t])], 1)] = t;
    for (int u = threadIdx.x; u < nt256; u += blockDim.x) {
        const unsigned m = tmask[2 * u] | ((2 * u + 1 < nt128) ? tmask[2 * u + 1] : 0u);
        order256[atomicAdd(&bins[1][32 - __popc(m)], 1)] = u;
    }
    for (int t = nt128 + threadIdx.x; t < cap128; t += blockDim.x) order128[t] = -1;
    for (int u = nt256 + threadIdx.x; u < cap256; u += blockDim.x) order256[u] = -1;
}

extern "C" int lb2_tile_order(void* handle, void* stream, const uint32_t* row_mask, const int32_t* row_perm, const int32_t* d_n, int32_t n_cap,
                              int32_t* order128, int32_t* order256, void* scratch) {
    Lb2Handle* h = (Lb2Handle*)handle;
    LB2_REQUIRE(h, h && row_mask && order128 && order256 && scratch && n_cap > 0, "tile_order");
    cudaStream_t s = (cudaStream_t)stream;
    const int cap128 = cdiv(n_cap, 128);
    k_tile_masks<<<cdiv(cap128, 8), 256, 0, s>>>(row_mask, row_perm, d_n, n_cap, (unsigned*)scratch);
    LB2_POST_LAUNCH(h, "k_tile_masks");
    k_tile_sort<<<1, 1024, 0, s>>>((const unsigned*)scratch, d_n, n_cap, order128, order256);
    LB2_POST_LAUNCH(h, "k_tile_sort");
    return LB2_OK;
}
```

### lidiff_b200/csrc/spconv_tc.cu

```cuda
#include "common.cuh"
#include <algorithm>
#include <stdlib.h>
#include "tc_common.cuh"

namespace tc {

constexpr int THREADS = 384;
constexpr int NUM_PRODUCER = 128;
constexpr int NUM_CONSUMER_WARPS = 8;
constexpr int STEP_BUDGET = 64;
constexpr int MAX_KVOL = 27;
constexpr int MAX_STAGES = 4;
constexpr int EPI_BATCH = 4;

struct Params {
    int c1, c2, cout, kvol;
    const unsigned char* wpacked;
    const float* scale;
    const float* shift;
    int relu;
    const int* nbr;
    long long nbr_stride;
    const int* d_mout;
    int mout_cap;
    const int* row_perm;
    const unsigned* row_mask;
    const int* tile_order;
    int stages, nchunks, group;
    int npass, nsplit;
    lb2_conv_io io[2];
};

constexpr int PRODUCER_REGS = 88;
constexpr int CONSUMER_REGS = 208;
static_assert(128 * PRODUCER_REGS + 256 * CONSUMER_REGS <= THREADS * 168, "register split exceeds the CTA's allocation");

struct TileInfo {
    int idx[MAX_KVOL * BM];
    int row[BM];
    uint32_t mask[4];
    int item;
    int pad[3];
};
constexpr int NUM_BARS = 3 * MAX_STAGES + 4;

template <int NC>
__global__ void __launch_bounds__(THREADS, 1) k_spconv_tc(const Params p) {
    extern __shared__ unsigned char smem_raw[];
    const int M = p.d_mout ? min(*p.d_mout, p.mout_cap) : p.mout_cap;
    const int warp = threadIdx.x >> 5, lane = threadIdx.x & 31;
    const int ctot = p.c1 + p.c2;
    const int S = p.stages;

    const uint32_t raw = smem_u32(smem_raw);
    const uint32_t base = (raw + 1023u) & ~1023u;
    unsigned char* gen = smem_raw + (base - raw);
    constexpr uint32_t b_tile = (uint32_t)NC * 128u;
    const uint32_t b_full = (uint32_t)p.cout * 128u;
    const uint32_t stage_bytes = 2u * A_TILE + 2u * b_tile;
    TileInfo* info = reinterpret_cast<TileInfo*>(gen + (size_t)S * stage_bytes);
    const uint32_t bar0 = smem_u32(info + 2);
    auto full_a = [&](int s) { return bar0 + 8u * s; };
    auto full_b = [&](int s) { return bar0 + 8u * (MAX_STAGES + s); };
    auto empty = [&](int s) { return bar0 + 8u * (2 * MAX_STAGES + s); };
    auto info_full = [&](int b) { return bar0 + 8u * (3 * MAX_STAGES + b); };
    auto info_empty = [&](int b) { return bar0 + 8u * (3 * MAX_STAGES + 2 + b); };

    if (threadIdx.x == 0) {
        for (int s = 0; s < S; ++s) { mbar_init(full_a(s), NUM_PRODUCER); mbar_init(full_b(s), 1); mbar_init(empty(s), NUM_CONSUMER_WARPS); }
        for (int b = 0; b < 2; ++b) { mbar_init(info_full(b), NUM_PRODUCER); mbar_init(info_empty(b), NUM_CONSUMER_WARPS); }
        asm volatile("fence.mbarrier_init.release.cluster;" ::: "memory");
    }
    __syncthreads();

    if (warpgroup_role() == 0) {
        setmaxnreg_dec<PRODUCER_REGS>();
        const int sub = threadIdx.x & 7;
        const int rbase = threadIdx.x >> 3;
        const int D = max(S - 2, 0);
        int it = 0, arrived = 0;
        auto tile_of = [&](int x) {
            const int slot_i = x / (p.nsplit * p.npass);
            return slot_i * BM >= p.mout_cap ? -1 : p.tile_order ? __ldg(p.tile_order + slot_i) : slot_i;
        };
        auto load_row = [&](int tile) {
            const int slot = tile * BM + threadIdx.x;
            return (tile >= 0 && slot < M) ? (p.row_perm ? __ldg(p.row_perm + slot) : slot) : -1;
        };
        auto load_indices = [&](int row, int (&v)[MAX_KVOL]) {
            const uint32_t want = row < 0 ? 0u : (p.row_mask ? __ldg(p.row_mask + row) : ~0u);
#pragma unroll
            for (int k = 0; k < MAX_KVOL; ++k) {
                v[k] = -1;
                if (k < p.kvol && ((want >> k) & 1u)) v[k] = p.nbr ? __ldg(p.nbr + (long long)k * p.nbr_stride + row) : row;
            }
        };
        int x = blockIdx.x, tile = tile_of(x), row = load_row(tile), v[MAX_KVOL];
        load_indices(row, v);
        for (int j = 0;; ++j) {
            TileInfo& ti = info[j & 1];
            mbar_wait(info_empty(j & 1), ((j >> 1) & 1) ^ 1);
            if (tile < 0 || tile * BM >= M) {
                if (threadIdx.x == 0) ti.item = -1;
                mbar_arrive(info_full(j & 1));
                break;
            }
            {
                ti.row[threadIdx.x] = row;
                uint32_t have = 0;
#pragma unroll
                for (int k = 0; k < MAX_KVOL; ++k) {
                    if (k < p.kvol) {
                        ti.idx[k * BM + threadIdx.x] = v[k];
                        if (v[k] >= 0) have |= 1u << k;
                    }
                }
                const uint32_t wmask = __reduce_or_sync(0xffffffffu, have);
                if (lane == 0) ti.mask[warp] = wmask;
                if (threadIdx.x == 0) ti.item = x;
            }
            mbar_arrive(info_full(j & 1));
            mbar_wait(info_full(j & 1), (j >> 1) & 1);
            const uint32_t kmask = ti.mask[0] | ti.mask[1] | ti.mask[2] | ti.mask[3];
            const int x_next = x + gridDim.x;
            const int tile_next = tile_of(x_next);
            const int n0 = (x % p.nsplit) * NC;
            const lb2_conv_io io = p.io[(x / p.nsplit) % p.npass];
            const bool use_h = (io.in1_h != nullptr) && (p.c2 == 0 || io.in2_h != nullptr);
            for (uint32_t km = kmask; km; km &= km - 1) {
                const int k = __ffs(km) - 1;
                const int* idxk = ti.idx + k * BM;
                int src[8];
#pragma unroll
                for (int r = 0; r < 8; ++r) src[r] = idxk[rbase + 16 * r];
                for (int c = 0; c < p.nchunks; ++c) {
                    const int s = it % S;
                    mbar_wait(empty(s), ((it / S) & 1) ^ 1);
                    unsigned char* a_hi = gen + (size_t)s * stage_bytes;
                    const uint32_t a_hi_u = base + (uint32_t)s * stage_bytes;
                    if (threadIdx.x == 0) {
                        const uint32_t dst = a_hi_u + 2u * A_TILE;
                        const unsigned char* wsrc = p.wpacked + PACK_HEADER + ((size_t)k * p.nchunks + c) * (2u * b_full) + (size_t)n0 * 128u;
                        mbar_expect_tx(full_b(s), 2u * b_tile);
                        bulk_g2s(dst, wsrc, b_tile, full_b(s));
                        bulk_g2s(dst + b_tile, wsrc + b_full, b_tile, full_b(s));
                    }
                    const int ch = c * KC + sub * 8;
                    if (ch < ctot) {
                        const bool first = ch < p.c1;
                        const int cw = first ? p.c1 : p.c2;
                        const int co = first ? ch : ch - p.c1;
                        if (use_h) produce_a_split(reinterpret_cast<const __half*>(first ? io.in1_h : io.in2_h), cw, co, src, a_hi_u, a_hi_u + A_TILE, rbase, sub);
                        else produce_a_f32(first ? io.in1 : io.in2, cw, co, src, a_hi, a_hi + A_TILE, rbase, sub);
                    }
                    cp_async_commit();
                    ++it;
                    if (it - arrived > D) {
                        cp_async_wait_dyn(D);
                        fence_proxy_async();
                        mbar_arrive(full_a(arrived % S));
                        ++arrived;
                    }
                }
            }
            const int s = it % S;
            mbar_wait(empty(s), ((it / S) & 1) ^ 1);
            if (threadIdx.x == 0) mbar_arrive(full_b(s));
            ++it;
            x = x_next;
            tile = tile_next;
            row = load_row(tile);
            cp_async_wait<0>();
            fence_proxy_async();
            for (; arrived < it; ++arrived) mbar_arrive(full_a(arrived % S));
            load_indices(row, v);
        }
    } else {
        setmaxnreg_inc<CONSUMER_REGS>();
        const int wg = (warp >> 2) - 1;
        const float out_scale = __ldg(reinterpret_cast<const float*>(p.wpacked) + 1);
        int it = 0;
        for (int j = 0;; ++j) {
            const TileInfo& ti = info[j & 1];
            mbar_wait(info_full(j & 1), (j >> 1) & 1);
            const int x = ti.item;
            if (x < 0) break;
            const int n_off = __popc(ti.mask[0] | ti.mask[1] | ti.mask[2] | ti.mask[3]);
            float acc[NC / 2], tot[NC / 2];
#pragma unroll
            for (int i = 0; i < NC / 2; ++i) tot[i] = -0.f;
            const int n_it = n_off * p.nchunks;
            int c = 0, in_group = 0, off_idx = 0, prev_s = -1;
            for (int i = 0; i < n_it; ++i, ++it) {
                const int s = it % S;
                const uint32_t par = (it / S) & 1;
                mbar_wait(full_b(s), par);
                mbar_wait(full_a(s), par);
                const uint32_t a_hi = base + (uint32_t)s * stage_bytes + (uint32_t)wg * (A_TILE / 2), a_lo = a_hi + A_TILE;
                const uint32_t b_hi = base + (uint32_t)s * stage_bytes + 2u * A_TILE, b_lo = b_hi + b_tile;
                const int ksteps = min(KC, ctot - c * KC) >> 4;
                reg_fence(acc);
                wg_stage_mma<NC>(acc, a_hi, a_lo, b_hi, b_lo, ksteps, in_group == 0 && c == 0);
                reg_fence(acc);
                wgmma_wait<1>();
                if (prev_s >= 0 && lane == 0) mbar_arrive(empty(prev_s));
                prev_s = s;
                if (++c < p.nchunks) continue;
                c = 0;
                ++off_idx;
                if (++in_group == p.group || off_idx == n_off) {
                    wgmma_wait<0>();
                    reg_fence(acc);
                    if (lane == 0) mbar_arrive(empty(prev_s));
                    prev_s = -1;
#pragma unroll
                    for (int i = 0; i < NC / 2; ++i) tot[i] = __fadd_rn(tot[i], acc[i]);
                    in_group = 0;
                }
            }
            wgmma_wait<0>();
            const int se = it % S;
            mbar_wait(full_b(se), (it / S) & 1);
            mbar_wait(full_a(se), (it / S) & 1);
            ++it;
            float* stage_c = reinterpret_cast<float*>(gen + (size_t)se * stage_bytes);
            {
                const int r0 = wg * 64 + (warp & 3) * 16 + (lane >> 2);
#pragma unroll
                for (int i = 0; i < NC / 2; i += 2) {
                    const int row = r0 + 8 * ((i >> 1) & 1), col = 8 * (i >> 2) + 2 * (lane & 3);
                    *reinterpret_cast<float2*>(stage_c + row * NC + (((col >> 2) ^ (row & 7)) << 2) + (col & 3)) =
                        make_float2(tot[i] * out_scale, tot[i + 1] * out_scale);
                }
            }
            asm volatile("bar.sync 1, 256;" ::: "memory");
            const lb2_conv_io io = p.io[(x / p.nsplit) % p.npass];
            const int n0 = (x % p.nsplit) * NC;
            const int cw = warp - 4;
            constexpr int nv = NC >> 2;
            constexpr int PER_LANE = (BM / NUM_CONSUMER_WARPS) * nv / 32;
            static_assert(PER_LANE % EPI_BATCH == 0, "a lane's elements come in whole batches");
            const bool has_res = io.residual || io.residual_h;
            const bool gated = io.out_gated || io.out_gated_h;
            const float4 zero4 = make_float4(0.f, 0.f, 0.f, 0.f);
            for (int e0 = 0; e0 < PER_LANE; e0 += EPI_BATCH) {
                int orow[EPI_BATCH], col[EPI_BATCH];
                long long gi[EPI_BATCH];
                float4 a4[EPI_BATCH], pre4[EPI_BATCH], s4[EPI_BATCH], h4[EPI_BATCH], res4[EPI_BATCH], g4[EPI_BATCH];
#pragma unroll
                for (int b = 0; b < EPI_BATCH; ++b) {
                    const int e = lane + 32 * (e0 + b);
                    const int rr = cw + NUM_CONSUMER_WARPS * (e / nv);
                    const int lcol = (e % nv) * 4;
                    col[b] = n0 + lcol;
                    orow[b] = ti.row[rr];
                    const bool live = orow[b] >= 0;
                    const long long ro = (long long)orow[b] * p.cout;
                    a4[b] = *reinterpret_cast<const float4*>(stage_c + rr * NC + (((lcol >> 2) ^ (rr & 7)) << 2));
                    pre4[b] = (live && io.pre_add) ? __ldg(reinterpret_cast<const float4*>(io.pre_add + ro + col[b])) : zero4;
                    s4[b] = p.scale ? __ldg(reinterpret_cast<const float4*>(p.scale + col[b])) : zero4;
                    h4[b] = p.scale ? __ldg(reinterpret_cast<const float4*>(p.shift + col[b])) : zero4;
                    res4[b] = (live && has_res) ? load_residual4(io.residual, io.residual_h, orow[b], p.cout, col[b]) : zero4;
                    gi[b] = (live && gated && io.gate_table && io.gate_idx) ? __ldg(io.gate_idx + orow[b]) : 0;
                }
#pragma unroll
                for (int b = 0; b < EPI_BATCH; ++b)
                    g4[b] = (orow[b] >= 0 && gated && io.gate_table) ? __ldg(reinterpret_cast<const float4*>(io.gate_table + gi[b] * p.cout + col[b])) : zero4;
#pragma unroll
                for (int b = 0; b < EPI_BATCH; ++b) {
                    if (orow[b] < 0) continue;
                    const long long ro = (long long)orow[b] * p.cout;
                    float y[4] = {a4[b].x, a4[b].y, a4[b].z, a4[b].w};
                    if (io.pre_add) {
                        y[0] += pre4[b].x; y[1] += pre4[b].y; y[2] += pre4[b].z; y[3] += pre4[b].w;
                    }
                    if (p.scale) {
                        y[0] = fmaf(y[0], s4[b].x, h4[b].x); y[1] = fmaf(y[1], s4[b].y, h4[b].y);
                        y[2] = fmaf(y[2], s4[b].z, h4[b].z); y[3] = fmaf(y[3], s4[b].w, h4[b].w);
                    }
                    if (has_res) {
                        y[0] += res4[b].x; y[1] += res4[b].y; y[2] += res4[b].z; y[3] += res4[b].w;
                    }
                    if (p.relu) {
#pragma unroll
                        for (int q = 0; q < 4; ++q) y[q] = fmaxf(y[q], 0.f);
                    }
                    if (io.out) *reinterpret_cast<float4*>(io.out + ro + col[b]) = make_float4(y[0], y[1], y[2], y[3]);
                    if (io.out_h) store_split4(io.out_h, orow[b], p.cout, col[b], y);
                    if (gated) {
                        if (io.gate_table) {
                            y[0] *= g4[b].x; y[1] *= g4[b].y; y[2] *= g4[b].z; y[3] *= g4[b].w;
                        }
                        if (io.out_gated) *reinterpret_cast<float4*>(io.out_gated + ro + col[b]) = make_float4(y[0], y[1], y[2], y[3]);
                        if (io.out_gated_h) store_split4(io.out_gated_h, orow[b], p.cout, col[b], y);
                    }
                }
            }
            fence_proxy_async();
            __syncwarp();
            if (lane == 0) {
                mbar_arrive(empty(se));
                mbar_arrive(info_empty(j & 1));
            }
        }
    }
}

__global__ void k_weight_absmax(const float* __restrict__ w, long long n, unsigned* __restrict__ header) {
    long long t = (long long)blockIdx.x * blockDim.x + threadIdx.x;
    float m = 0.f;
    for (; t < n; t += (long long)gridDim.x * blockDim.x) m = fmaxf(m, fabsf(w[t]));
#pragma unroll
    for (int o = 16; o > 0; o >>= 1) m = fmaxf(m, __shfl_xor_sync(0xffffffffu, m, o));
    if ((threadIdx.x & 31) == 0) atomicMax(header, __float_as_uint(m));
}

__device__ __forceinline__ float weight_scale(unsigned max_bits) {
    const float m = __uint_as_float(max_bits);
    if (!(m > 0.f) || !isfinite(m)) return 1.f;
    int e;
    frexpf(m, &e);
    return ldexpf(1.f, min(14 - e, 126));
}

__global__ void k_pack_weights(const float* __restrict__ w, int kvol, int cin, int cout, int nchunks, unsigned char* __restrict__ out) {
    const long long total = (long long)kvol * nchunks * cout * KC;
    long long t = (long long)blockIdx.x * blockDim.x + threadIdx.x;
    const float scale = weight_scale(*reinterpret_cast<const unsigned*>(out));
    if (t == 0) reinterpret_cast<float*>(out)[1] = 1.0f / scale;
    if (t >= total) return;
    const int kk = (int)(t % KC);
    const int n = (int)((t / KC) % cout);
    const int c = (int)((t / ((long long)KC * cout)) % nchunks);
    const int k = (int)(t / ((long long)KC * cout * nchunks));
    const int ch = c * KC + kk;
    const float v = ch < cin ? w[((long long)k * cin + ch) * cout + n] * scale : 0.f;
    const __half hi = __float2half_rn(v);
    const __half lo = __float2half_rn(v - __half2float(hi));
    const size_t tile = (size_t)cout * 128;
    unsigned char* blob = out + PACK_HEADER + ((size_t)k * nchunks + c) * 2 * tile;
    const uint32_t off = sw128(n, kk >> 3) + (uint32_t)(kk & 7) * 2u;
    *reinterpret_cast<__half*>(blob + off) = hi;
    *reinterpret_cast<__half*>(blob + tile + off) = lo;
}

static bool shape_ok(int c1, int c2, int cout, int kvol) {
    const int ctot = c1 + c2;
    if (kvol < 1 || kvol > MAX_KVOL) return false;
    if (ctot % 16 != 0 || ctot < 16) return false;
    if (c2 > 0 && (c1 % 8 != 0 || c2 % 8 != 0)) return false;
    if (cout % 32 != 0 || cout < 32 || cout > 256) return false;
    if (cout > 128 && cout != 256) return false;
    return true;
}

static size_t smem_bytes(int nc, int stages) {
    return 1024 + (size_t)stages * (2 * A_TILE + 2 * (size_t)nc * 128) + 2 * sizeof(TileInfo) + NUM_BARS * sizeof(uint64_t);
}

template <int NC>
static int launch(Lb2Handle* h, cudaStream_t s, const Params& p, int stages) {
    const size_t smem = smem_bytes(NC, stages);
    cudaError_t e = lb2_configure_smem(h, LB2_K_TC + (NC / 32 - 1), k_spconv_tc<NC>, (int)(227 * 1024));
    if (e != cudaSuccess) return lb2_fail(h, LB2_ERR_CUDA, "k_spconv_tc smem attribute: %s", cudaGetErrorString(e));
    const unsigned grid = (unsigned)std::min<long long>(h->num_sms, (long long)cdiv(p.mout_cap, BM) * p.npass * p.nsplit);
    k_spconv_tc<NC><<<grid, THREADS, smem, s>>>(p);
    LB2_POST_LAUNCH(h, "k_spconv_tc");
    return LB2_OK;
}

}

bool lb2_spconv_tc_supported(const lb2_conv_desc* d) { return tc::shape_ok(d->c1, d->c2, d->cout, d->kvol); }

extern "C" size_t lb2_packed_weight_bytes(int32_t kvol, int32_t cin, int32_t cout) {
    if (!tc::shape_ok(cin, 0, cout, kvol)) return 0;
    const int nchunks = (cin + tc::KC - 1) / tc::KC;
    return tc::PACK_HEADER + (size_t)kvol * nchunks * 2 * (size_t)cout * 128;
}

extern "C" int lb2_pack_weights(void* handle, void* stream, const float* weight, int32_t kvol, int32_t cin, int32_t cout, void* packed) {
    Lb2Handle* h = (Lb2Handle*)handle;
    LB2_REQUIRE(h, h && weight && packed, "pack_weights null");
    if (!tc::shape_ok(cin, 0, cout, kvol)) return lb2_fail(h, LB2_ERR_UNSUP, "pack_weights: shape not supported by the tensor-core variant%s", "");
    const int nchunks = (cin + tc::KC - 1) / tc::KC;
    const long long total = (long long)kvol * nchunks * cout * tc::KC;
    const long long nw = (long long)kvol * cin * cout;
    if (cudaMemsetAsync(packed, 0, tc::PACK_HEADER, (cudaStream_t)stream) != cudaSuccess) return lb2_fail(h, LB2_ERR_CUDA, "pack_weights memset%s", "");
    tc::k_weight_absmax<<<(unsigned)std::min<long long>(cdiv(nw, 256), 1024), 256, 0, (cudaStream_t)stream>>>(weight, nw, (unsigned*)packed);
    LB2_POST_LAUNCH(h, "k_weight_absmax");
    tc::k_pack_weights<<<cdiv(total, 256), 256, 0, (cudaStream_t)stream>>>(weight, kvol, cin, cout, nchunks, (unsigned char*)packed);
    LB2_POST_LAUNCH(h, "k_pack_weights");
    return LB2_OK;
}

int lb2_spconv_tc_launch(Lb2Handle* h, cudaStream_t s, const lb2_conv_desc* d) {
    tc::Params p;
    p.c1 = d->c1; p.c2 = d->c2; p.cout = d->cout; p.kvol = d->kvol;
    p.wpacked = (const unsigned char*)d->weight_packed;
    p.scale = d->scale; p.shift = d->shift; p.relu = d->relu;
    p.nbr = d->nbr; p.nbr_stride = d->nbr_stride; p.d_mout = d->d_mout; p.mout_cap = d->mout_cap; p.row_perm = d->row_perm;
    p.tile_order = d->nbr ? d->tile_order128 : nullptr;
    p.row_mask = d->nbr ? (const unsigned*)d->row_mask : nullptr;
    p.nchunks = (d->c1 + d->c2 + tc::KC - 1) / tc::KC;
    const int nsplit = d->cout > 128 ? 2 : 1;
    const int nc = d->cout / nsplit;
    p.npass = d->npass > 1 ? 2 : 1;
    p.nsplit = nsplit;
    int stages = tc::MAX_STAGES;
    while (stages > 2 && tc::smem_bytes(nc, stages) > 227 * 1024) --stages;
    p.stages = stages;
    const int steps_per_offset = 3 * ((d->c1 + d->c2 + 15) / 16);
    p.group = std::max(1, tc::STEP_BUDGET / steps_per_offset);
    p.io[0] = d->io[0]; p.io[1] = d->io[d->npass > 1 ? 1 : 0];
    switch (nc) {
        case 32: return tc::launch<32>(h, s, p, stages);
        case 64: return tc::launch<64>(h, s, p, stages);
        case 96: return tc::launch<96>(h, s, p, stages);
        case 128: return tc::launch<128>(h, s, p, stages);
        default: return lb2_fail(h, LB2_ERR_UNSUP, "tensor-core variant: no kernel for %s output channels per CTA", nc == 80 ? "80" : nc == 112 ? "112" : "this many");
    }
}
```

### lidiff_b200/engine.py

```python
from __future__ import annotations

import math
import os
from collections import ChainMap

import numpy as np
import torch

from . import _lib
from ._lib import ConvDesc, ConvIO, DpmCoef, ScatterDesc
from .scheduler import DPMSolverMultistepScheduler

GATE_NAMES = ("stage1", "stage2", "stage3", "stage4", "up1", "up2", "up3", "up4")
GATE_LEVEL = (0, 1, 2, 3, 4, 3, 2, 1)
BN_EPS = 1e-5


class ConvLayer:

    def __init__(self, h, sd, pconv, pbn, device):
        W = sd[f"{pconv}.kernel"].detach().to(device=device, dtype=torch.float32)
        if W.dim() == 2:
            W = W[None]
        self.W = W.contiguous()
        self.kvol, self.cin, self.cout = self.W.shape
        self.name = pconv
        if pbn is not None:
            g = lambda k: sd[f"{pbn}.bn.{k}"].detach().to(device=device, dtype=torch.float32)
            scale = g("weight") / torch.sqrt(g("running_var") + BN_EPS)
            self.scale = scale.contiguous()
            self.shift = (g("bias") - g("running_mean") * scale).contiguous()
        else:
            self.scale = self.shift = None
        self.Wp = h.pack_weights(self.W)
        self.Wc = self.Wpc = None
        if self.kvol == 27 and self.Wp is not None and h.scatter_supported(self.cin, 0, self.cout, 27):
            self.Wc = self.W[13:14].contiguous()
            self.Wpc = h.pack_weights(self.Wc)


class Linear:
    def __init__(self, sd, p, device, cols=None):
        w = sd[f"{p}.weight"].detach().to(device=device, dtype=torch.float32)
        self.w = (w if cols is None else w[:, cols[0]:cols[1]]).contiguous()
        self.b = sd[f"{p}.bias"].detach().to(device=device, dtype=torch.float32).contiguous()
        self.n_out, self.n_in = self.w.shape


class Act:
    __slots__ = ("f", "h", "P", "cap", "C")

    def __init__(self, P, cap, C, f, h):
        self.P, self.cap, self.C, self.f, self.h = P, cap, C, f, h


def _ptr(t, p):
    return None if t is None else t[min(p, t.shape[0] - 1)].data_ptr()


def _net_layers(h, sd, device, decoder: bool):
    L = {}

    def add(pconv, pbn):
        L[pconv] = ConvLayer(h, sd, pconv, pbn, device)

    def res(p):
        add(f"{p}.net.0", f"{p}.net.1")
        add(f"{p}.net.3", f"{p}.net.4")
        if f"{p}.downsample.0.kernel" in sd:
            add(f"{p}.downsample.0", f"{p}.downsample.1")

    add("stem.0", "stem.1")
    add("stem.3", "stem.4")
    for n in range(1, 5):
        add(f"stage{n}.0.net.0", f"stage{n}.0.net.1")
        res(f"stage{n}.1")
        res(f"stage{n}.2")
    if decoder:
        for n in range(1, 5):
            add(f"up{n}.0.net.0", f"up{n}.0.net.1")
            res(f"up{n}.1.0")
            res(f"up{n}.1.1")
    return L


class Geometry:

    def __init__(self, h, n_cap: int, with_up: bool = True, levels: int = 5, use_pairs: bool = True):
        dev = h.device
        self.h, self.n_cap, self.levels, self.use_pairs = h, n_cap, levels, use_pairs
        i32 = dict(dtype=torch.int32, device=dev)
        self.C = [torch.zeros((n_cap, 4), **i32) for _ in range(levels)]
        self.d_n = [torch.zeros(1, **i32) for _ in range(levels)]
        self.grid = [h.new_grid(n_cap) for _ in range(levels)]
        self.inv = [torch.zeros(n_cap, **i32) for _ in range(levels)]
        self.nbr3 = [torch.empty((27, n_cap), **i32) for _ in range(levels)]
        self.nbr_dn = [None] + [torch.empty((8, n_cap), **i32) for _ in range(levels - 1)]
        self.nbr_up = [torch.empty((8, n_cap), **i32) for _ in range(levels - 1)] + [None] if with_up else None
        self.scratch = h.unique_scratch(n_cap)
        self.voxel_scratch = h.voxel_mean_scratch(n_cap, 3)
        self.pairs = torch.zeros(18, dtype=torch.int64, device=dev)
        self.map_id = {}
        self.mask_of = {}
        self.ro_scratch = torch.zeros((h.row_order_scratch_bytes(n_cap) + 3) // 4, **i32)
        self.ro_scratch_late = self.to_scratch_late = None
        self.perm3 = [torch.zeros(n_cap, **i32) for _ in range(levels)]
        self.perm_dn = [None] + [torch.zeros(n_cap, **i32) for _ in range(levels - 1)]
        self.perm_up = [torch.zeros(n_cap, **i32) for _ in range(levels - 1)] + [None] if with_up else None
        self.perm_of = {}
        self.use_tile_order = os.environ.get("LB2_TILE_ORDER", "1") != "0"
        self.map_self = os.environ.get("LB2_MAP_SELF", "1") != "0"
        self.tile_order_of = {}
        self.to_scratch = torch.zeros((n_cap + 127) // 128, **i32)
        self.morton_levels = set(int(c) for c in os.environ.get("LB2_MORTON_LEVELS", "") if c.isdigit())
        self.pair_levels = min(3, levels)
        self.pair_level_set = set(int(c) for c in os.environ.get("LB2_SCATTER_LEVELS", "") if c.isdigit())
        self.pairs_of = {}
        self.pl_scratch = torch.zeros(64, **i32)
        want = [use_pairs and l in self.pair_level_set for l in range(self.pair_levels)]
        self.pair_in = [torch.zeros(26 * n_cap, **i32) if w else None for w in want]
        self.pair_out = [torch.zeros(26 * n_cap, **i32) if w else None for w in want]
        self.koff = [torch.zeros(28, **i32) for _ in range(self.pair_levels)]
        self.tile_off = [torch.zeros(28, **i32) for _ in range(self.pair_levels)]

    def build(self, coords_f: torch.Tensor, n_points: int, after_levels=None, late_stream=None, late_done=None):
        h, N = self.h, self.n_cap
        h.unique_build(coords_f, None, None, n_points, 0, self.grid[0], self.C[0], self.inv[0], self.d_n[0], self.scratch)
        for l in range(1, self.levels):
            h.unique_build(None, self.C[l - 1], self.d_n[l - 1], N, 1 << l, self.grid[l], self.C[l], self.inv[l], self.d_n[l], self.scratch)
        if after_levels is not None:
            after_levels()
        self.pairs.zero_()

        def one(grid, l_out, ks, step, nbr, perm, slot, ro_scratch=None, to_scratch=None):
            ro_scratch = self.ro_scratch if ro_scratch is None else ro_scratch
            to_scratch = self.to_scratch if to_scratch is None else to_scratch
            mask = self.mask_of.get(nbr.data_ptr())
            if mask is None:
                mask = self.mask_of[nbr.data_ptr()] = torch.zeros(N, dtype=torch.int32, device=nbr.device)
            if ks == 3 and self.map_self:
                h.kernel_map_self(grid, self.C[l_out], self.d_n[l_out], N, step, nbr, N, self.pairs[slot:slot + 1], mask)
            else:
                h.kernel_map(grid, self.C[l_out], self.d_n[l_out], N, ks, step, nbr, N, self.pairs[slot:slot + 1], mask)
            morton = ks == 3 and l_out in self.morton_levels
            h.row_order(mask, self.d_n[l_out], N, ks ** 3, perm, ro_scratch, self.C[l_out] if morton else None, l_out)
            if self.use_tile_order:
                to = self.tile_order_of.get(nbr.data_ptr())
                if to is None:
                    to = self.tile_order_of[nbr.data_ptr()] = (torch.zeros((N + 127) // 128, dtype=torch.int32, device=nbr.device),
                                                               torch.zeros((N + 255) // 256, dtype=torch.int32, device=nbr.device))
                h.tile_order(mask, perm, self.d_n[l_out], N, to[0], to[1], to_scratch)
            self.map_id[nbr.data_ptr()] = slot
            self.perm_of[nbr.data_ptr()] = perm

        def map3(l, **kw):
            one(self.grid[l], l, 3, 1 << l, self.nbr3[l], self.perm3[l], l, **kw)
            if l < self.pair_levels and self.use_pairs and l in self.pair_level_set:
                h.pair_list(self.nbr3[l], N, self.d_n[l], N, 27, 13, self.pair_in[l], self.pair_out[l], self.koff[l], self.tile_off[l], self.pl_scratch)
                self.pairs_of[self.nbr3[l].data_ptr()] = l

        def map_dn(l, **kw):
            one(self.grid[l - 1], l, 2, 1 << (l - 1), self.nbr_dn[l], self.perm_dn[l], 4 + l, **kw)

        def map_up(l, **kw):
            one(self.grid[l + 1], l, 2, -(1 << l), self.nbr_up[l], self.perm_up[l], 9 + l, **kw)

        split = late_stream is not None and self.levels >= 3 and not (self.use_pairs and self.pair_level_set)
        early3 = (0, 1) if split else tuple(range(self.levels))
        early_dn = (1,) if split else tuple(range(1, self.levels))
        if split:
            if self.ro_scratch_late is None:
                self.ro_scratch_late, self.to_scratch_late = torch.zeros_like(self.ro_scratch), torch.zeros_like(self.to_scratch)
            kw = dict(ro_scratch=self.ro_scratch_late, to_scratch=self.to_scratch_late)
            late_stream.wait_stream(torch.cuda.current_stream())
            with torch.cuda.stream(late_stream):
                for l in range(2, self.levels):
                    map_dn(l, **kw)
                    map3(l, **kw)
                if self.nbr_up is not None:
                    for l in range(self.levels - 2, -1, -1):
                        map_up(l, **kw)
                late_done.record(late_stream)
        for l in early3:
            if l >= 1 and l in early_dn:
                map_dn(l)
            map3(l)
        for l in early_dn:
            if l not in early3:
                map_dn(l)
        if not split and self.nbr_up is not None:
            for l in range(self.levels - 1):
                map_up(l)

    def voxel_mean(self, feats, n_points, out):
        assert feats.shape[1] == 3, "voxel_scratch is sized for 3-channel point features"
        self.h.voxel_mean(feats, self.inv[0], n_points, 3, self.d_n[0], self.n_cap, out, self.voxel_scratch)

    def sizes(self):
        return [int(d.item()) for d in self.d_n]


class _PairLookup:

    def __init__(self, geom):
        self.geom = geom

    def get(self, ptr):
        l = self.geom.pairs_of.get(ptr)
        return None if l is None else (self.geom, l)


class DenoiseEngine:
    def __init__(self, sd_enc: dict, sd_diff: dict, *, device="cuda", n_points=180000, denoising_steps=50,
                 cond_weight=6.0, resolution=0.05, t_steps=1000, beta_start=3.5e-5, beta_end=0.007,
                 div_mode=1, conv_algo=_lib.ALGO_AUTO, batch_coord=0.0, sd_refine: dict | None = None, max_range=50.0, batch=1):
        self.device = torch.device(device)
        self.N = int(n_points)
        self.B = int(batch)
        self.cap = self.B * self.N
        if self.B != 1:
            _check_batch(self.B, self.N, self.device)
        self.h = _lib.get_handle(self.device)
        self._bcol = None if self.B == 1 else \
            torch.arange(self.B, dtype=torch.float32, device=self.device).repeat_interleave(self.N).contiguous()
        self.w = float(cond_weight)
        self.resolution = float(resolution)
        self.div_mode = int(div_mode)
        self.conv_algo = conv_algo
        h, dev = self.h, self.device
        self.enc = _net_layers(h, sd_enc, dev, decoder=False)
        self.diff = _net_layers(h, sd_diff, dev, decoder=True)
        self.refine = _net_layers(h, sd_refine, dev, decoder=True) if sd_refine is not None else None
        self.refine_head = (Linear(sd_refine, "last.0", dev), Linear(sd_refine, "last.2", dev)) if sd_refine is not None else None
        self.max_range = float(max_range)
        self.sched = DPMSolverMultistepScheduler(num_train_timesteps=t_steps, beta_start=beta_start, beta_end=beta_end,
                                                 beta_schedule="linear", algorithm_type="sde-dpmsolver++", solver_order=2)
        self.sched.set_timesteps(denoising_steps)
        self.T = len(self.sched.timesteps)
        self.latent = [(Linear(sd_diff, f"latent_{g}.0", dev), Linear(sd_diff, f"latent_{g}.2", dev)) for g in GATE_NAMES]
        self.temp = [(Linear(sd_diff, f"{g}_temp.0", dev), Linear(sd_diff, f"{g}_temp.2", dev)) for g in GATE_NAMES]
        self.lat_p, self.lat_t, self.lat_2 = [], [], []
        for g in GATE_NAMES:
            half = sd_diff[f"latemp_{g}.0.weight"].shape[1] // 2
            pc, tc = ((half, 2 * half), (0, half)) if g == "up1" else ((0, half), (half, 2 * half))
            self.lat_p.append(Linear(sd_diff, f"latemp_{g}.0", dev, cols=pc))
            self.lat_t.append(Linear(sd_diff, f"latemp_{g}.0", dev, cols=tc))
            self.lat_2.append(Linear(sd_diff, f"latemp_{g}.2", dev))
        self.head = (Linear(sd_diff, "last.0", dev), Linear(sd_diff, "last.2", dev))
        self._bufs = {}
        self._graphs = {}
        self.use_row_order = True
        self.use_scatter = True
        self.use_split = True
        self.lean = os.environ.get("LB2_LEAN", "1") != "0" and not os.environ.get("LB2_SCATTER_LEVELS")
        self._acts = {}
        self._perm_lookup = {}
        self._tile_order_lookup = {}
        self.geom = Geometry(h, self.cap, with_up=True)
        self._perm_lookup = self.geom.perm_of
        self._mask_lookup = self.geom.mask_of
        self._tile_order_lookup = self.geom.tile_order_of
        self._pairs_lookup = _PairLookup(self.geom)
        self.geom_cond = None
        self.part_cap = 0
        self.nn_algo = os.environ.get("LB2_NN_ALGO", "tree")
        self.use_side_stream = os.environ.get("LB2_SIDE_STREAM", "1") != "0" and torch.cuda.is_available() and self.device.type == "cuda"
        if self.use_side_stream:
            self._side = torch.cuda.Stream(device=self.device)
            self._side_done = torch.cuda.Event()
            self._side2 = torch.cuda.Stream(device=self.device)
            self._side2_done = torch.cuda.Event()
            self._side3 = torch.cuda.Stream(device=self.device)
            self._side3_done = torch.cuda.Event()
        self.late_maps = self.use_side_stream and os.environ.get("LB2_LATE_MAPS", "1") != "0"
        self.conv_events = None
        self.layer_log = None
        self.pair_hist = None
        self._hist_row = 0
        self._conv_counter = 0
        self._have_x0 = False
        self.use_graphs = os.environ.get("LB2_GRAPHS", "1") != "0" and torch.cuda.is_available() and self.device.type == "cuda"
        self._graphs = {}
        self._eager_steps = 0
        self.graph_replays = 0
        self.replayed_launches = 0
        self._captured_launches = 0
        self._prepare_time_tables()
        self._prepare_uncond()

    @classmethod
    def from_modules(cls, pipe, **kw):
        sd_e = {k: v for k, v in pipe.partial_enc.state_dict().items()}
        sd_d = {k: v for k, v in pipe.model.state_dict().items()}
        hp = pipe.hparams
        if getattr(pipe, "model_refine", None) is not None:
            kw.setdefault("sd_refine", {k: v for k, v in pipe.model_refine.state_dict().items()})
        kw.setdefault("max_range", hp["data"].get("max_range", 50.0))
        return cls(sd_e, sd_d, device=pipe.device, n_points=hp["data"]["num_points"], denoising_steps=hp["diff"]["s_steps"],
                   cond_weight=pipe.w_uncond, resolution=hp["data"]["resolution"], t_steps=hp["diff"]["t_steps"],
                   beta_start=hp["diff"]["beta_start"], beta_end=hp["diff"]["beta_end"], **kw)

    def buf(self, name, shape, dtype=torch.float32):
        t = self._bufs.get(name)
        if t is None or tuple(t.shape) != tuple(shape) or t.dtype != dtype:
            if t is not None:
                self._graphs.clear()
            t = torch.zeros(shape, dtype=dtype, device=self.device)
            self._bufs[name] = t
        return t

    def act(self, name, P, cap, C, f32=True, split=True) -> Act:
        split = bool(split and self.use_split and self.conv_algo != _lib.ALGO_FFMA and C % 8 == 0)
        f32 = bool(f32 or not split)
        a = self._acts.get(name)
        if a is None or (a.P, a.cap, a.C) != (P, cap, C) or (a.f is not None) != f32 or (a.h is not None) != split:
            if a is not None:
                self._graphs.clear()
            f = torch.zeros((P, cap, C), dtype=torch.float32, device=self.device) if f32 else None
            hh = torch.zeros((P, cap, 2 * C), dtype=torch.float16, device=self.device) if split else None
            a = self._acts[name] = Act(P, cap, C, f, hh)
        return a

    def _linear(self, x, lin: Linear, out, act=0, m_cap=None, d_m=None, prebias=None, pre_act=0, bias=True):
        m_cap = x.shape[0] if m_cap is None else m_cap
        self.h.linear(x, x.stride(0), lin.w, lin.b if bias else None, None, 0, m_cap, d_m, lin.n_in, lin.n_out, act,
                      out, out.stride(0), prebias, pre_act)
        return out

    def _head(self, x, head, out, out_act, d_m):
        l0, l1 = head
        self.h.head_mlp(x, x.stride(1), x.stride(0), l0.w, l0.b, l1.w, l1.b, x.shape[1], d_m, l0.n_in, l0.n_out, l1.n_out, out_act,
                        x.shape[0], out, out.stride(1), out.stride(0))

    def _timestep_embedding(self, ts: torch.Tensor) -> torch.Tensor:
        half = 48
        freq = torch.from_numpy(np.exp(np.arange(0, half) * -(np.log(10000) / (half - 1)))).float().to(self.device)
        arg = ts.to(self.device)[:, None] * freq[None, :]
        return torch.cat([torch.sin(arg), torch.cos(arg)], dim=1).contiguous()

    def _prepare_time_tables(self):
        T, dev = self.T, self.device
        temb = self._timestep_embedding(self.sched.timesteps)
        self.bvec = []
        for g in range(8):
            l0, l2 = self.temp[g]
            u = self._linear(temb, l0, torch.empty((T, l0.n_out), device=dev), act=1)
            tv = self._linear(u, l2, torch.empty((T, l2.n_out), device=dev))
            self.bvec.append(self._linear(tv, self.lat_t[g], torch.empty((T, self.lat_t[g].n_out), device=dev)))

    def _gate_tables(self, A_list, rows_cap, d_rows, step, tag):
        out = []
        for g in range(8):
            t = self.buf(f"gate_{tag}_{g}", (rows_cap, self.lat_2[g].n_out))
            self._linear(A_list[g], self.lat_2[g], t, m_cap=rows_cap, d_m=d_rows, prebias=self.bvec[g][step], pre_act=1)
            out.append(t)
        return out

    def _part_A(self, part_F, rows_cap, d_rows, tag):
        A = []
        for g in range(8):
            l0, l2 = self.latent[g]
            h1 = self._linear(part_F, l0, self.buf(f"lat_h_{tag}", (rows_cap, l0.n_out)), act=1, m_cap=rows_cap, d_m=d_rows)
            p = self._linear(h1, l2, self.buf(f"lat_p_{tag}", (rows_cap, l2.n_out)), m_cap=rows_cap, d_m=d_rows)
            a = self.buf(f"lat_A_{tag}_{g}", (rows_cap, self.lat_p[g].n_out))
            A.append(self._linear(p, self.lat_p[g], a, m_cap=rows_cap, d_m=d_rows, bias=False))
        return A

    def _conv(self, lay: ConvLayer, nbr, d_m, cap, in1: Act, in2: Act = None, out: Act = None, residual: Act = None, relu=True,
              gate=None, out_gated: Act = None, npass=1):
        d = ConvDesc()
        d.c1 = in1.C
        d.c2 = in2.C if in2 is not None else 0
        assert d.c1 + d.c2 == lay.cin, (d.c1, d.c2, lay.cin)
        f = lambda a: None if a is None else a.f
        hh = lambda a: None if a is None else a.h
        pre = None
        geom_lvl = self._pairs_lookup.get(nbr.data_ptr()) if (nbr is not None and self.use_scatter and lay.Wpc is not None
                                                               and self.conv_algo != _lib.ALGO_FFMA) else None
        if geom_lvl is not None:
            g, l = geom_lvl
            pre = self.buf(f"scatter.{lay.cout}", (2, cap, lay.cout))
            sd = ScatterDesc()
            sd.c1, sd.c2, sd.cout, sd.kvol = d.c1, d.c2, lay.cout, 27
            sd.weight_packed = lay.Wp.data_ptr()
            sd.pair_in, sd.pair_out = g.pair_in[l].data_ptr(), g.pair_out[l].data_ptr()
            sd.koff, sd.tile_off = g.koff[l].data_ptr(), g.tile_off[l].data_ptr()
            sd.npass = npass
            for p in range(npass):
                sd.in1[p], sd.in2[p], sd.out[p] = _ptr(f(in1), p), _ptr(f(in2), p), pre[p].data_ptr()
                sd.in1_h[p], sd.in2_h[p] = _ptr(hh(in1), p), _ptr(hh(in2), p)
            sd.d_zero_rows, sd.zero_rows_cap = d_m.data_ptr(), cap
        else:
            sd = None
        map_ptr = nbr.data_ptr() if nbr is not None else None
        d.cout, d.kvol = lay.cout, (1 if pre is not None else lay.kvol)
        d.weight = (lay.Wc if pre is not None else lay.W).data_ptr()
        wp = lay.Wpc if pre is not None else lay.Wp
        d.weight_packed = wp.data_ptr() if wp is not None else None
        d.scale = lay.scale.data_ptr() if lay.scale is not None else None
        d.shift = lay.shift.data_ptr() if lay.shift is not None else None
        d.relu = 1 if relu else 0
        if pre is not None:
            nbr = None
        d.nbr = nbr.data_ptr() if nbr is not None else None
        d.nbr_stride = nbr.stride(0) if nbr is not None else cap
        d.d_mout = d_m.data_ptr() if d_m is not None else None
        d.mout_cap, d.npass = cap, npass
        perm = self._perm_lookup.get(nbr.data_ptr()) if (nbr is not None and self.use_row_order) else None
        d.row_perm = perm.data_ptr() if perm is not None else None
        mask = self._mask_lookup.get(nbr.data_ptr()) if nbr is not None else None
        d.row_mask = mask.data_ptr() if mask is not None else None
        to = self._tile_order_lookup.get(nbr.data_ptr()) if (nbr is not None and perm is not None) else None
        d.tile_order128 = to[0].data_ptr() if to is not None else None
        d.tile_order256 = to[1].data_ptr() if to is not None else None
        res_h = hh(residual) if (residual is not None and residual.f is None) else None
        for p in range(npass):
            gt = gi = None
            if gate is not None:
                gt = gate[p][0].data_ptr()
                gi = gate[p][1].data_ptr() if gate[p][1] is not None else None
            d.io[p] = ConvIO(_ptr(f(in1), p), _ptr(f(in2), p), _ptr(f(residual), p), _ptr(f(out), p), gt, gi, _ptr(f(out_gated), p),
                             pre[p].data_ptr() if pre is not None else None,
                             _ptr(hh(in1), p), _ptr(hh(in2), p), _ptr(hh(out), p), _ptr(hh(out_gated), p), _ptr(res_h, p))
        if self.layer_log is not None:
            self.layer_log.append(dict(name=lay.name, scatter=sd is not None, map=map_ptr, d_m=d_m.data_ptr() if d_m is not None else None,
                                       cin=lay.cin, cout=lay.cout, kvol=lay.kvol, npass=npass,
                                       tc=bool(lay.Wp is not None and self.conv_algo != _lib.ALGO_FFMA)))
        if self.conv_events is not None:
            e0, e1 = torch.cuda.Event(enable_timing=True), torch.cuda.Event(enable_timing=True)
            e0.record()
            if sd is not None:
                self.h.spconv_scatter(sd)
            self.h.spconv(d, self.conv_algo)
            e1.record()
            self.conv_events.append((e0, e1, self._conv_counter))
            self._conv_counter += 1
        else:
            if sd is not None:
                self.h.spconv_scatter(sd)
            self.h.spconv(d, self.conv_algo)

    def _res(self, L, p, geom, lvl, in1: Act, in2: Act, npass, tag, gate=None, want_plain=True, lean=False, out_f32=False):
        cap = geom.n_cap
        nbr, d_m = geom.nbr3[lvl], geom.d_n[lvl]
        cmid = L[f"{p}.net.0"].cout
        hbuf = self.act(f"{tag}.h", npass, cap, cmid, f32=not lean)
        self._conv(L[f"{p}.net.0"], nbr, d_m, cap, in1, in2, out=hbuf, npass=npass)
        if f"{p}.downsample.0" in L:
            sbuf = self.act(f"{tag}.s", npass, cap, cmid, split=not lean)
            self._conv(L[f"{p}.downsample.0"], None, d_m, cap, in1, in2, out=sbuf, relu=False, npass=npass)
        else:
            assert in2 is None
            sbuf = in1
        out = self.act(f"{tag}.o", npass, cap, cmid, f32=(not lean) or out_f32) if want_plain else None
        og = self.act(f"{tag}.g", npass, cap, cmid, f32=not lean) if gate is not None else None
        self._conv(L[f"{p}.net.3"], nbr, d_m, cap, hbuf, None, out=out, residual=sbuf, relu=True, gate=gate, out_gated=og, npass=npass)
        return out, og

    def _encoder(self, L, geom, F0: Act, npass, tag, gates=None, lean=False, before_gates=None, before_stage2=None):
        cap = geom.n_cap
        s0 = self.act(f"{tag}.stem0", 1, cap, 32, f32=not lean)
        self._conv(L["stem.0"], geom.nbr3[0], geom.d_n[0], cap, F0, out=s0, npass=1)
        x0 = self.act(f"{tag}.x0", 1, cap, 32, f32=(not lean) or gates is not None)
        self._conv(L["stem.3"], geom.nbr3[0], geom.d_n[0], cap, s0, out=x0, npass=1)
        skips = [x0]
        if gates is not None:
            if before_gates is not None:
                before_gates()
            cur = self.act(f"{tag}.x0g", npass, cap, 32, f32=not lean)
            for p in range(npass):
                tb, ix = gates[0][p]
                self.h.gate_mul(x0.f[0], tb, ix, geom.d_n[0], cap, 32, cur.f[p] if cur.f is not None else None,
                                cur.h[p] if cur.h is not None else None)
        else:
            cur = x0
        for n in range(1, 5):
            if n == 2 and before_stage2 is not None:
                before_stage2()
            a = self.act(f"{tag}.s{n}a", npass, cap, L[f"stage{n}.0.net.0"].cout, f32=not lean)
            self._conv(L[f"stage{n}.0.net.0"], geom.nbr_dn[n], geom.d_n[n], cap, cur, out=a, npass=npass)
            b, _ = self._res(L, f"stage{n}.1", geom, n, a, None, npass, f"{tag}.s{n}r1", lean=lean)
            g = gates[n] if gates is not None else None
            x, xg = self._res(L, f"stage{n}.2", geom, n, b, None, npass, f"{tag}.s{n}r2", gate=g, lean=lean)
            skips.append(x)
            cur = xg if gates is not None else x
        return skips, cur

    def _decoder(self, L, geom, skips, cur: Act, npass, tag, gates, lean=False):
        cap = geom.n_cap
        y = cur
        for n in range(1, 5):
            lvl = 4 - n
            d = self.act(f"{tag}.u{n}d", npass, cap, L[f"up{n}.0.net.0"].cout, f32=not lean)
            self._conv(L[f"up{n}.0.net.0"], geom.nbr_up[lvl], geom.d_n[lvl], cap, y, out=d, npass=npass)
            b, _ = self._res(L, f"up{n}.1.0", geom, lvl, d, skips[lvl], npass, f"{tag}.u{n}r1", lean=lean)
            g = gates[4 + n] if (gates is not None and n < 4) else None
            o, og = self._res(L, f"up{n}.1.1", geom, lvl, b, None, npass, f"{tag}.u{n}r2", gate=g, want_plain=(g is None), lean=lean,
                              out_f32=(n == 4))
            y = og if g is not None else o
        return y

    def _prepare_uncond(self):
        dev = self.device
        g1 = Geometry(self.h, 16, with_up=False, use_pairs=False)
        coords = torch.zeros((16, 4), dtype=torch.float32, device=dev)
        g1.build(coords, 16)
        F0 = self.act("uenc.F0", 1, 16, 3)
        F0.f.zero_()
        skips, _ = self._encoder(self.enc, g1, F0, 1, "uenc")
        part_u = skips[4].f[0][:1].clone()
        A = self._part_A(part_u, 1, None, "u")
        self.table_u = []
        for g in range(8):
            t = torch.empty((self.T, self.lat_2[g].n_out), device=dev)
            for s in range(self.T):
                self._linear(A[g], self.lat_2[g], t[s:s + 1], prebias=self.bvec[g][s], pre_act=1)
            self.table_u.append(t)
        for k in [k for k in self._acts if k.startswith("uenc")]:
            del self._acts[k]

    def set_condition(self, scan: torch.Tensor):
        dev = self.device
        pts = scan.reshape(-1, 3).to(device=dev, dtype=torch.float32).contiguous()
        N = pts.shape[0]
        if self.geom_cond is None or self.geom_cond.n_cap != N:
            self._graphs.clear()
            self.geom_cond = Geometry(self.h, N, with_up=False, use_pairs=False)
            self._perm_lookup = ChainMap(self.geom.perm_of, self.geom_cond.perm_of)
            self._mask_lookup = ChainMap(self.geom.mask_of, self.geom_cond.mask_of)
            self._tile_order_lookup = ChainMap(self.geom.tile_order_of, self.geom_cond.tile_order_of)
        coords = self.buf("cond.coords", (N, 4))
        coords[:, 0] = 0 if self._bcol is None else self._bcol
        self.h.quantize(pts, self.resolution, self.div_mode, self.buf("cond.q", (N, 3)))
        coords[:, 1:] = self._bufs["cond.q"]
        g = self.geom_cond
        g.build(coords, N)
        F0 = self.act("cond.F0", 1, N, 3)
        g.voxel_mean(pts, N, F0.f[0])
        skips, _ = self._encoder(self.enc, g, F0, 1, "cenc")
        self.part_F = skips[4].f[0]
        self.part_C, self.part_dn, self.part_grid = g.C[4], g.d_n[4], g.grid[4]
        self.part_cap = N
        self.part_tree = self.h.nn_tree(self.part_C, self.part_dn, N, out=getattr(self, "part_tree", None))
        self.A_cond = self._part_A(self.part_F, N, self.part_dn, "c")

    def step(self, i: int, x_t, x_next, coords, coords_next, x_init, noise_i, x0_state, eps_out=None):
        h, N, g = self.h, self.cap, self.geom
        self._conv_counter = 0
        nn = [None] * 5
        tabs_box = []

        def gate_tables():
            tabs_box.append(self._gate_tables(self.A_cond, self.part_cap, self.part_dn, i, "c"))

        if self.use_side_stream:
            self._side2.wait_stream(torch.cuda.current_stream())
            with torch.cuda.stream(self._side2):
                gate_tables()
                self._side2_done.record(self._side2)
        else:
            gate_tables()

        def matches():
            for l in range(4, -1, -1):
                ix = self.buf(f"nn{l}", (N,), torch.int32)
                if self.nn_algo == "grid":
                    h.nn_match_grid(g.C[l], g.d_n[l], N, self.part_C, self.part_dn, self.part_cap, self.part_grid, 16, 4, ix)
                elif l == 4:
                    h.nn_match_tree(g.C[l], g.d_n[l], N, self.part_tree, self.part_cap, ix)
                else:
                    h.nn_match_tree(g.C[l], g.d_n[l], N, self.part_tree, self.part_cap, ix, self.part_C, g.inv[l + 1], nn[l + 1])
                nn[l] = ix

        def after_levels():
            if not self.use_side_stream:
                return matches()
            main = torch.cuda.current_stream()
            self._side.wait_stream(main)
            with torch.cuda.stream(self._side):
                matches()
                self._side_done.record(self._side)

        def join_sides():
            if self.use_side_stream:
                torch.cuda.current_stream().wait_event(self._side_done)
                torch.cuda.current_stream().wait_event(self._side2_done)

        def join_late_maps():
            if self.late_maps:
                torch.cuda.current_stream().wait_event(self._side3_done)

        if self.late_maps:
            g.build(coords, N, after_levels, late_stream=self._side3, late_done=self._side3_done)
        else:
            g.build(coords, N, after_levels)
        if self.pair_hist is not None:
            if self.late_maps:
                torch.cuda.current_stream().wait_event(self._side3_done)
            g.pairs[13:18] = torch.cat(g.d_n).long()
            self.pair_hist[self._hist_row % self.pair_hist.shape[0]] = g.pairs
            self._hist_row += 1
        F0 = self.act("F0", 1, N, 3)
        g.voxel_mean(x_t, N, F0.f[0])
        tabs_c = tabs_box[0]
        gates = [[(tabs_c[k], nn[GATE_LEVEL[k]]), (self.table_u[k][i:i + 1], None)] for k in range(8)]
        skips, cur = self._encoder(self.diff, g, F0, 2, "d", gates, lean=self.lean, before_gates=join_sides, before_stage2=join_late_maps)
        y4 = self._decoder(self.diff, g, skips, cur, 2, "d", gates, lean=self.lean)
        eps = self.buf("eps_vox", (2, N, 3))
        self._head(y4.f, self.head, eps, 0, g.d_n[0])
        c = self.sched.coefficients(i)
        second = self._have_x0 and not (i == self.T - 1 and self.T < 15)
        self._have_x0 = True
        cf = DpmCoef(c["c_sample"], c["c_x0"], c["c_noise"], c["sigma_s"], c["alpha_s"], c["inv_r0"] if second else 0.0,
                     self.w, self.resolution, 1 if second else 0, self.div_mode, 1)
        h.guidance_dpm_step(eps[0], eps[1], g.inv[0], x_t, x_init, noise_i, x0_state, N, cf, eps_out, x_next, coords_next, self._bcol)

    def start(self, x_init: torch.Tensor, x_feats: torch.Tensor, fresh: bool = True):
        dev, N = self.device, self.cap
        if fresh:
            self._have_x0 = False
        x_src = x_init.reshape(-1, 3)
        assert x_src.shape[0] == N, f"engine built for {N} points, got {x_src.shape[0]}"
        x_init = self.buf("x_init", (N, 3), torch.float64)
        x_init.copy_(x_src)
        self.set_condition(x_init)
        st = dict(x_init=x_init, xa=self.buf("x_a", (N, 3)), xb=self.buf("x_b", (N, 3)), ca=self.buf("c_a", (N, 4)),
                  cb=self.buf("c_b", (N, 4)), x0s=self.buf("x0_state", (N, 3), torch.float64), i=0)
        st["xa"].copy_(x_feats.reshape(-1, 3).to(device=dev, dtype=torch.float32))
        st["ca"][:, 0] = 0 if self._bcol is None else self._bcol
        self.h.quantize(st["xa"], self.resolution, self.div_mode, self.buf("q0", (N, 3)))
        st["ca"][:, 1:] = self._bufs["q0"]
        return st

    def advance(self, st, noise_i, host_noise=None, host_out=None):
        i = st["i"] % self.T
        graphed = self.use_graphs and self.conv_events is None and self.layer_log is None and self.pair_hist is None
        if host_noise is not None or graphed:
            nbuf = self.buf("noise_in", (self.cap, 3))
            nbuf.copy_(host_noise if host_noise is not None else noise_i, non_blocking=True)
            noise_i = nbuf
        if not graphed or self._eager_steps < 1:
            self.step(i, st["xa"], st["xb"], st["ca"], st["cb"], st["x_init"], noise_i, st["x0s"])
            self._eager_steps += 1
        else:
            second = self._have_x0 and not (i == self.T - 1 and self.T < 15)
            key = (i, st["xa"].data_ptr(), bool(second))
            ent = self._graphs.get(key)
            if ent is None:
                have = self._have_x0
                l0 = self.h.launch_count()
                g = torch.cuda.CUDAGraph()
                with torch.cuda.graph(g):
                    self.step(i, st["xa"], st["xb"], st["ca"], st["cb"], st["x_init"], noise_i, st["x0s"])
                ent = self._graphs[key] = (g, self.h.launch_count() - l0)
                self._captured_launches += ent[1]
                self._have_x0 = have
            ent[0].replay()
            self._have_x0 = True
            self.graph_replays += 1
            self.replayed_launches += ent[1]
        st["xa"], st["xb"], st["ca"], st["cb"] = st["xb"], st["xa"], st["cb"], st["ca"]
        st["i"] += 1
        if host_out is not None:
            host_out.copy_(st["xa"], non_blocking=True)

    def launches(self) -> int:
        return self.h.launch_count() - self._captured_launches + self.replayed_launches

    def run(self, x_init: torch.Tensor, x_feats: torch.Tensor, step_noise=None, n_steps=None, return_device=False, fresh=True):
        dev, N = self.device, self.N
        st = self.start(x_init, x_feats, fresh=fresh)
        T = self.T if n_steps is None else n_steps
        if step_noise is not None:
            step_noise = step_noise.reshape(-1, self.cap, 3).to(device=dev, dtype=torch.float32).contiguous()
        for i in range(T):
            nz = step_noise[i] if step_noise is not None else torch.randn((self.B, N, 3), device=dev, dtype=torch.float32).reshape(-1, 3)
            self.advance(st, nz)
        if return_device:
            return st["xa"]
        out = st["xa"].cpu().numpy()
        if self.h.read_status() & 1:
            raise RuntimeError("lidiff_b200: a coordinate left the supported key range during sampling")
        return out

    def postprocess(self, completed: torch.Tensor, x_init: torch.Tensor) -> torch.Tensor:
        x, y, z = completed[:, 0], completed[:, 1], completed[:, 2]
        dist = torch.sqrt((x * x + y * y) + z * z)
        zi = x_init.reshape(-1, 3)[:, 2]
        max_z = zi.max().item()
        min_z = (zi.mean() - 2 * zi.std()).item()
        keep = (dist < self.max_range) & (z < max_z) & (z > min_z)
        return completed[keep].contiguous()

    def refine_offsets(self, pts: torch.Tensor, batch_col: torch.Tensor | None = None) -> torch.Tensor:
        if self.refine is None:
            raise RuntimeError("DenoiseEngine was built without the refinement network (sd_refine)")
        h, g, N = self.h, self.geom, self.cap
        pts = pts.to(device=self.device, dtype=torch.float32).contiguous()
        n = pts.shape[0]
        if n > N:
            raise RuntimeError(f"refine_offsets: {n} points exceed the engine capacity {N}")
        if n == 0:
            return torch.zeros((0, 18), device=self.device)
        coords = self.buf("r.coords", (N, 4))
        q = self.buf("r.q", (N, 3))
        h.quantize(pts, self.resolution, self.div_mode, q[:n])
        coords[:n, 0] = 0 if batch_col is None else batch_col
        coords[:n, 1:] = q[:n]
        g.build(coords, n)
        F0 = self.act("r.F0", 1, N, 3)
        g.voxel_mean(pts, n, F0.f[0])
        skips, cur = self._encoder(self.refine, g, F0, 1, "r", lean=self.lean)
        y4 = self._decoder(self.refine, g, skips, cur, 1, "r", None, lean=self.lean)
        off_v = self.buf("r.off_v", (1, N, 18))
        self._head(y4.f, self.refine_head, off_v, 2, g.d_n[0])
        off_v = off_v[0]
        out = torch.empty((n, 18), device=self.device)
        h.gather_rows(off_v, g.inv[0], n, 18, out)
        return out

    def complete(self, x_init: torch.Tensor, x_feats: torch.Tensor, step_noise=None, fresh=True):
        x_t = self.run(x_init, x_feats, step_noise, return_device=True, fresh=fresh)
        post = self.postprocess(x_t, x_init.reshape(-1, 3).to(self.device))
        off = self.refine_offsets(post).reshape(-1, 6, 3)
        refined = (post[:, None, :] + off).reshape(-1, 3)
        if self.h.read_status() & 1:
            raise RuntimeError("lidiff_b200: a coordinate left the supported key range during sampling")
        return refined, post

    def postprocess_batch(self, completed: torch.Tensor, x_init: torch.Tensor):
        B, N = self.B, self.N
        x, y, z = completed[:, 0], completed[:, 1], completed[:, 2]
        dist = torch.sqrt((x * x + y * y) + z * z)
        zi = x_init.reshape(B, N, 3)
        max_z = torch.stack([zi[b, :, 2].max() for b in range(B)]).float()
        min_z = torch.stack([zi[b, :, 2].mean() - 2 * zi[b, :, 2].std() for b in range(B)]).float()
        keep = ((dist < self.max_range).reshape(B, N) & (z.reshape(B, N) < max_z[:, None]) & (z.reshape(B, N) > min_z[:, None])).reshape(-1)
        return completed[keep].contiguous(), self._bcol[keep].contiguous(), keep.reshape(B, N).sum(1)

    def complete_batch(self, x_init: torch.Tensor, x_feats: torch.Tensor, step_noise=None, fresh=True):
        if self.B == 1:
            return [self.complete(x_init, x_feats, step_noise, fresh=fresh)]
        x_t = self.run(x_init, x_feats, step_noise, return_device=True, fresh=fresh)
        post, bcol, counts = self.postprocess_batch(x_t, x_init.to(self.device))
        off = self.refine_offsets(post, bcol).reshape(-1, 6, 3)
        refined = (post[:, None, :] + off).reshape(-1, 3)
        if self.h.read_status() & 1:
            raise RuntimeError("lidiff_b200: a coordinate left the supported key range during sampling")
        counts = counts.tolist()
        return list(zip(refined.split([6 * c for c in counts]), post.split(counts)))


ENGINE_BYTES_PER_ROW = 120_000
MAX_BATCH = 1 << 10


def _check_batch(B: int, n_points: int, device):
    if not 1 <= B <= MAX_BATCH:
        raise RuntimeError(f"DenoiseEngine: batch={B} is outside 1..{MAX_BATCH} (coordinate keys carry 10 batch bits)")
    rows = B * n_points
    if 27 * rows >= 1 << 31:
        raise RuntimeError(f"DenoiseEngine: batch={B} x {n_points} points = {rows} rows exceed the 32-bit kernel-map index range")
    if device.type == "cuda" and torch.cuda.is_available():
        free, _ = torch.cuda.mem_get_info(device)
        free += torch.cuda.memory_reserved(device) - torch.cuda.memory_allocated(device)
        need = rows * ENGINE_BYTES_PER_ROW
        if need > free:
            raise RuntimeError(f"DenoiseEngine: batch={B} x {n_points} points needs about {need / 2**30:.1f} GiB of device memory, "
                               f"{free / 2**30:.1f} GiB are free")
```

Before: 28.44.

## Split wide 27-offset sparse convs into offset-range passes with partial accumulation

Deep-level sparse convolutions (stage4, up1, up2) with large channel counts are split into two or three launches, each covering a contiguous range of kernel offsets. Each pass uses its own row permutation and tile order, sorted by the offset mask within that range, and accumulates into an fp32 partial buffer that the next pass reads. The intent is to make tiles denser in active offsets and cut wasted MMA work on sparse rows. The cost is extra launches, extra sorting passes at geometry build time, and the partial buffer round trips through global memory.

```diff
diff --git a/include/lidiff_b200.h b/include/lidiff_b200.h
--- a/include/lidiff_b200.h
+++ b/include/lidiff_b200.h
@@ -54,6 +54,12 @@
 
 int lb2_tile_order(void* h, void* stream, const uint32_t* row_mask, const int32_t* row_perm, const int32_t* d_n, int32_t n_cap,
                    int32_t* order128, int32_t* order256, void* scratch);
+
+int lb2_row_order_range(void* h, void* stream, const uint32_t* row_mask, const int32_t* d_n, int32_t n_cap, int32_t k0, int32_t k1,
+                        int32_t* perm, int32_t* d_live, void* scratch);
+
+int lb2_tile_order_range(void* h, void* stream, const uint32_t* row_mask, const int32_t* row_perm, const int32_t* d_n, int32_t n_cap,
+                         int32_t k0, int32_t k1, int32_t* order128, void* scratch);
 
 typedef struct {
     const float*   in1;
@@ -88,6 +94,9 @@
     lb2_conv_io    io[2];
     const int32_t* tile_order128;
     const int32_t* tile_order256;
+    int32_t        k0, k1;
+    const float*   partial_in;
+    float*         partial_out;
 } lb2_conv_desc;
 
 #define LB2_ALGO_AUTO  0
diff --git a/lidiff_b200/_lib.py b/lidiff_b200/_lib.py
--- a/lidiff_b200/_lib.py
+++ b/lidiff_b200/_lib.py
@@ -30,7 +30,8 @@
                 ("d_mout", C.c_void_p), ("mout_cap", C.c_int32), ("row_perm", C.c_void_p), ("row_mask", C.c_void_p),
                 ("npass", C.c_int32),
                 ("io", ConvIO * 2),
-                ("tile_order128", C.c_void_p), ("tile_order256", C.c_void_p)]
+                ("tile_order128", C.c_void_p), ("tile_order256", C.c_void_p),
+                ("k0", C.c_int32), ("k1", C.c_int32), ("partial_in", C.c_void_p), ("partial_out", C.c_void_p)]
 
 
 class ScatterDesc(C.Structure):
@@ -51,7 +52,7 @@
 
 EXPORTS = [
     "lb2_create", "lb2_destroy", "lb2_last_error", "lb2_version", "lb2_launch_count", "lb2_read_status",
-    "lb2_tile_order",
+    "lb2_tile_order", "lb2_row_order_range", "lb2_tile_order_range",
     "lb2_quantize", "lb2_unique_scratch_bytes", "lb2_unique_build", "lb2_voxel_mean_scratch_bytes", "lb2_voxel_mean", "lb2_kernel_map",
     "lb2_spconv_forward", "lb2_packed_weight_bytes", "lb2_pack_weights", "lb2_nn_match", "lb2_linear",
     "lb2_gate_mul", "lb2_gather_rows", "lb2_head_mlp", "lb2_kernel_map_self", "lb2_guidance_dpm_step", "lb2_farthest_point_sample",
@@ -109,6 +110,8 @@
         d.lb2_kernel_map_self.argtypes = [vp, vp, Grid, vp, vp, i32, i32, vp, i64, vp, vp]
         d.lb2_row_order.argtypes = [vp, vp, vp, vp, i32, i32, vp, vp, vp, i32]
         d.lb2_tile_order.argtypes = [vp, vp, vp, vp, vp, i32, vp, vp, vp]
+        d.lb2_row_order_range.argtypes = [vp, vp, vp, vp, i32, i32, i32, vp, vp, vp]
+        d.lb2_tile_order_range.argtypes = [vp, vp, vp, vp, vp, i32, i32, i32, vp, vp]
         d.lb2_row_order_scratch_bytes.restype = C.c_size_t
         d.lb2_row_order_scratch_bytes.argtypes = [i32]
         d.lb2_spconv_forward.argtypes = [vp, vp, C.POINTER(ConvDesc), C.c_int]
@@ -241,6 +244,14 @@
         self._check(self.dll.lb2_tile_order(self.hp, self._stream(), _ptr(row_mask), _ptr(row_perm), _ptr(d_n), int(n_cap), _ptr(order128),
                                             _ptr(order256), _ptr(scratch)), "lb2_tile_order")
 
+    def row_order_range(self, row_mask, d_n, n_cap, k0, k1, perm, d_live, scratch):
+        self._check(self.dll.lb2_row_order_range(self.hp, self._stream(), _ptr(row_mask), _ptr(d_n), int(n_cap), int(k0), int(k1), _ptr(perm),
+                                                 _ptr(d_live), _ptr(scratch)), "lb2_row_order_range")
+
+    def tile_order_range(self, row_mask, row_perm, d_n, n_cap, k0, k1, order128, scratch):
+        self._check(self.dll.lb2_tile_order_range(self.hp, self._stream(), _ptr(row_mask), _ptr(row_perm), _ptr(d_n), int(n_cap), int(k0), int(k1),
+                                                  _ptr(order128), _ptr(scratch)), "lb2_tile_order_range")
+
     def spconv(self, desc: ConvDesc, algo: int = ALGO_AUTO):
         self._check(self.dll.lb2_spconv_forward(self.hp, self._stream(), C.byref(desc), int(algo)), "lb2_spconv_forward")
 
diff --git a/lidiff_b200/csrc/api.cu b/lidiff_b200/csrc/api.cu
--- a/lidiff_b200/csrc/api.cu
+++ b/lidiff_b200/csrc/api.cu
@@ -25,6 +25,11 @@
     }
     LB2_REQUIRE(h, d->c2 == 0 || d->c1 % 16 == 0, "c1 must be a multiple of 16 when in2 is given");
     cudaStream_t s = (cudaStream_t)stream;
+    if (d->k1 > 0) {
+        if (algo == LB2_ALGO_FFMA || !d->weight_packed || !lb2_spconv_tc_supported(d))
+            return lb2_fail(h, LB2_ERR_UNSUP, "an offset range needs the tensor-core variant%s", "");
+        return lb2_spconv_tc_launch(h, s, d);
+    }
     if (algo == LB2_ALGO_TC || algo == LB2_ALGO_TC_TILE) {
         if (!d->weight_packed || !lb2_spconv_tc_supported(d))
             return lb2_fail(h, LB2_ERR_UNSUP, "tensor-core variant does not support this layer%s", "");
diff --git a/lidiff_b200/csrc/coords.cu b/lidiff_b200/csrc/coords.cu
--- a/lidiff_b200/csrc/coords.cu
+++ b/lidiff_b200/csrc/coords.cu
@@ -473,6 +473,20 @@
     return ((__popc(extras) >= 2) ? (1u << 26) : 0u) | k26;
 }
 
+__device__ __host__ __forceinline__ int ro_range_nb(int k0, int k1) { return (k1 - k0) - ((k0 <= 13 && 13 < k1) ? 1 : 0); }
+__device__ __host__ __forceinline__ unsigned ro_range_mask(int k0, int k1) { return ((1u << k1) - 1u) & ~((1u << k0) - 1u); }
+__device__ __forceinline__ unsigned ro_key_range(unsigned mask, int k0, int k1) {
+    const unsigned sub = mask & ro_range_mask(k0, k1);
+    const int nb = ro_range_nb(k0, k1);
+    unsigned local = sub >> k0;
+    if (k0 <= 13 && 13 < k1) {
+        const int c = 13 - k0;
+        local = ((local >> (c + 1)) << c) | (local & ((1u << c) - 1u));
+    }
+    const unsigned multi = __popc(sub & ~(1u << 13)) >= 2 ? 1u : 0u;
+    return ((sub == 0u ? 1u : 0u) << (nb + 1)) | (multi << nb) | local;
+}
+
 __device__ __forceinline__ unsigned ro_part9(unsigned v) {
     v &= 0x1ffu;
     v = (v | (v << 16)) & 0x030000ffu;
@@ -490,7 +504,7 @@
     const unsigned* mask;
     const int4* coords;
     const int* vals;
-    int mode, coord_shift;
+    int mode, coord_shift, k0, k1;
 };
 __device__ __forceinline__ unsigned rs_key(const RsSrc& s, int i) {
     switch (s.mode) {
@@ -498,6 +512,7 @@
         case 1: return ro_key27(s.mask[i]);
         case 2: return ro_morton(s.coords[i], s.coord_shift);
         case 4: return s.mask[i] & 0xffu;
+        case 5: return ro_key_range(s.mask[i], s.k0, s.k1);
         default: return ro_key27(s.mask[s.vals[i]]);
     }
 }
@@ -629,6 +644,49 @@
     LB2_POST_LAUNCH(h, "k_rs_hist");
     k_rs_scatter<<<nblk, 32 * RS_WARPS, 0, s>>>(src, d_n, n_cap, 0, hist, total, nullptr, perm);
     LB2_POST_LAUNCH(h, "k_rs_scatter");
+    return LB2_OK;
+}
+
+__global__ void __launch_bounds__(256) k_range_live(const unsigned* __restrict__ mask, const int* __restrict__ d_n, int n_cap, unsigned rmask,
+                                                    int* __restrict__ d_live) {
+    const int n = d_n ? min(*d_n, n_cap) : n_cap;
+    const int i = blockIdx.x * blockDim.x + threadIdx.x;
+    const unsigned live = __ballot_sync(0xffffffffu, i < n && (__ldg(mask + i) & rmask) != 0u);
+    if ((threadIdx.x & 31) == 0 && live) atomicAdd(d_live, __popc(live));
+}
+
+extern "C" int lb2_row_order_range(void* handle, void* stream, const uint32_t* row_mask, const int32_t* d_n, int32_t n_cap, int32_t k0, int32_t k1,
+                                   int32_t* perm, int32_t* d_live, void* scratch) {
+    Lb2Handle* h = (Lb2Handle*)handle;
+    LB2_REQUIRE(h, h && row_mask && perm && d_live && scratch && n_cap > 0, "row_order_range");
+    LB2_REQUIRE(h, 0 <= k0 && k0 < k1 && k1 <= 27, "row_order_range: offset range outside [0, 27)");
+    cudaStream_t s = (cudaStream_t)stream;
+    const int nblk = rs_blocks(n_cap);
+    int* hist = (int*)scratch;
+    int* total = hist + (size_t)RS_BINS * nblk;
+    unsigned* keys_a = (unsigned*)(total + 6 * RS_BINS);
+    unsigned* keys_b = keys_a + n_cap;
+    int* vals_a = (int*)(keys_b + n_cap);
+    const int npass = cdiv(ro_range_nb(k0, k1) + 2, RS_BITS);
+    if (cudaMemsetAsync(total, 0, (size_t)npass * RS_BINS * sizeof(int), s) != cudaSuccess ||
+        cudaMemsetAsync(d_live, 0, sizeof(int32_t), s) != cudaSuccess)
+        return lb2_fail(h, LB2_ERR_CUDA, "row_order_range memset%s", "");
+    k_range_live<<<cdiv(n_cap, 256), 256, 0, s>>>(row_mask, d_n, n_cap, ro_range_mask(k0, k1), d_live);
+    LB2_POST_LAUNCH(h, "k_range_live");
+    for (int pass = 0; pass < npass; ++pass) {
+        const bool to_perm = ((npass - 1 - pass) & 1) == 0;
+        RsSrc src;
+        src.mask = row_mask; src.coords = nullptr; src.coord_shift = 0; src.k0 = k0; src.k1 = k1;
+        src.keys = (pass & 1) ? keys_a : keys_b;
+        src.vals = (pass == 0) ? nullptr : (to_perm ? vals_a : perm);
+        src.mode = (pass == 0) ? 5 : 0;
+        unsigned* kout = (pass == npass - 1) ? nullptr : ((pass & 1) ? keys_b : keys_a);
+        int* vout = to_perm ? perm : vals_a;
+        k_rs_hist<<<nblk, 256, 0, s>>>(src, d_n, n_cap, pass * RS_BITS, hist, total + pass * RS_BINS);
+        LB2_POST_LAUNCH(h, "k_rs_hist");
+        k_rs_scatter<<<nblk, 32 * RS_WARPS, 0, s>>>(src, d_n, n_cap, pass * RS_BITS, hist, total + pass * RS_BINS, kout, vout);
+        LB2_POST_LAUNCH(h, "k_rs_scatter");
+    }
     return LB2_OK;
 }
 
@@ -808,7 +866,7 @@
 }
 
 __global__ void __launch_bounds__(256) k_tile_masks(const unsigned* __restrict__ mask, const int* __restrict__ perm, const int* __restrict__ d_n,
-                                                    int n_cap, unsigned* __restrict__ tmask) {
+                                                    int n_cap, unsigned kmask, unsigned* __restrict__ tmask) {
     const int n = d_n ? min(*d_n, n_cap) : n_cap;
     const int nt = (n + 127) >> 7;
     const int warp = (blockIdx.x * blockDim.x + threadIdx.x) >> 5, lane = threadIdx.x & 31;
@@ -820,7 +878,7 @@
         if (slot < n) m |= __ldg(mask + (perm ? __ldg(perm + slot) : slot));
     }
     m = __reduce_or_sync(0xffffffffu, m);
-    if (lane == 0) tmask[warp] = m;
+    if (lane == 0) tmask[warp] = m & kmask;
 }
 
 __global__ void __launch_bounds__(1024) k_tile_sort(const unsigned* __restrict__ tmask, const int* __restrict__ d_n, int n_cap,
@@ -832,7 +890,7 @@
     if (threadIdx.x < 66) (&bins[0][0])[threadIdx.x] = 0;
     __syncthreads();
     for (int t = threadIdx.x; t < nt128; t += blockDim.x) atomicAdd(&bins[0][32 - __popc(tmask[t])], 1);
-    for (int u = threadIdx.x; u < nt256; u += blockDim.x) {
+    for (int u = threadIdx.x; order256 && u < nt256; u += blockDim.x) {
         const unsigned m = tmask[2 * u] | ((2 * u + 1 < nt128) ? tmask[2 * u + 1] : 0u);
         atomicAdd(&bins[1][32 - __popc(m)], 1);
     }
@@ -843,12 +901,12 @@
     }
     __syncthreads();
     for (int t = threadIdx.x; t < nt128; t += blockDim.x) order128[atomicAdd(&bins[0][32 - __popc(tmask[t])], 1)] = t;
-    for (int u = threadIdx.x; u < nt256; u += blockDim.x) {
+    for (int u = threadIdx.x; order256 && u < nt256; u += blockDim.x) {
         const unsigned m = tmask[2 * u] | ((2 * u + 1 < nt128) ? tmask[2 * u + 1] : 0u);
         order256[atomicAdd(&bins[1][32 - __popc(m)], 1)] = u;
     }
     for (int t = nt128 + threadIdx.x; t < cap128; t += blockDim.x) order128[t] = -1;
-    for (int u = nt256 + threadIdx.x; u < cap256; u += blockDim.x) order256[u] = -1;
+    for (int u = nt256 + threadIdx.x; order256 && u < cap256; u += blockDim.x) order256[u] = -1;
 }
 
 extern "C" int lb2_tile_order(void* handle, void* stream, const uint32_t* row_mask, const int32_t* row_perm, const int32_t* d_n, int32_t n_cap,
@@ -857,9 +915,23 @@
     LB2_REQUIRE(h, h && row_mask && order128 && order256 && scratch && n_cap > 0, "tile_order");
     cudaStream_t s = (cudaStream_t)stream;
     const int cap128 = cdiv(n_cap, 128);
-    k_tile_masks<<<cdiv(cap128, 8), 256, 0, s>>>(row_mask, row_perm, d_n, n_cap, (unsigned*)scratch);
+    k_tile_masks<<<cdiv(cap128, 8), 256, 0, s>>>(row_mask, row_perm, d_n, n_cap, 0xffffffffu, (unsigned*)scratch);
     LB2_POST_LAUNCH(h, "k_tile_masks");
     k_tile_sort<<<1, 1024, 0, s>>>((const unsigned*)scratch, d_n, n_cap, order128, order256);
     LB2_POST_LAUNCH(h, "k_tile_sort");
     return LB2_OK;
 }
+
+extern "C" int lb2_tile_order_range(void* handle, void* stream, const uint32_t* row_mask, const int32_t* row_perm, const int32_t* d_n, int32_t n_cap,
+                                    int32_t k0, int32_t k1, int32_t* order128, void* scratch) {
+    Lb2Handle* h = (Lb2Handle*)handle;
+    LB2_REQUIRE(h, h && row_mask && order128 && scratch && n_cap > 0, "tile_order_range");
+    LB2_REQUIRE(h, 0 <= k0 && k0 < k1 && k1 <= 27, "tile_order_range: offset range outside [0, 27)");
+    cudaStream_t s = (cudaStream_t)stream;
+    const int cap128 = cdiv(n_cap, 128);
+    k_tile_masks<<<cdiv(cap128, 8), 256, 0, s>>>(row_mask, row_perm, d_n, n_cap, ro_range_mask(k0, k1), (unsigned*)scratch);
+    LB2_POST_LAUNCH(h, "k_tile_masks");
+    k_tile_sort<<<1, 1024, 0, s>>>((const unsigned*)scratch, d_n, n_cap, order128, nullptr);
+    LB2_POST_LAUNCH(h, "k_tile_sort");
+    return LB2_OK;
+}
diff --git a/lidiff_b200/csrc/spconv_tc.cu b/lidiff_b200/csrc/spconv_tc.cu
--- a/lidiff_b200/csrc/spconv_tc.cu
+++ b/lidiff_b200/csrc/spconv_tc.cu
@@ -29,6 +29,9 @@
     int stages, nchunks, group;
     int npass, nsplit;
     lb2_conv_io io[2];
+    uint32_t range_mask, prior_mask;
+    const float* partial_in;
+    float* partial_out;
 };
 
 constexpr int PRODUCER_REGS = 88;
@@ -39,6 +42,7 @@
     int idx[MAX_KVOL * BM];
     int row[BM];
     uint32_t mask[4];
+    uint32_t prior[4];
     int item;
     int pad[3];
 };
@@ -87,13 +91,15 @@
             const int slot = tile * BM + threadIdx.x;
             return (tile >= 0 && slot < M) ? (p.row_perm ? __ldg(p.row_perm + slot) : slot) : -1;
         };
-        auto load_indices = [&](int row, int (&v)[MAX_KVOL]) {
-            const uint32_t want = row < 0 ? 0u : (p.row_mask ? __ldg(p.row_mask + row) : ~0u);
+        auto load_indices = [&](int& row, int (&v)[MAX_KVOL]) {
+            const uint32_t m = row < 0 ? 0u : (p.row_mask ? __ldg(p.row_mask + row) : ~0u);
+            const uint32_t want = m & p.range_mask;
 #pragma unroll
             for (int k = 0; k < MAX_KVOL; ++k) {
                 v[k] = -1;
-                if (k < p.kvol && ((want >> k) & 1u)) v[k] = p.nbr ? __ldg(p.nbr + (long long)k * p.nbr_stride + row) : row;
-            }
+                if (k < p.kvol && (want >> k) & 1u) v[k] = p.nbr ? __ldg(p.nbr + (long long)k * p.nbr_stride + row) : row;
+            }
+            if (m & p.prior_mask) row |= 1 << 30;
         };
         int x = blockIdx.x, tile = tile_of(x), row = load_row(tile), v[MAX_KVOL];
         load_indices(row, v);
@@ -106,7 +112,7 @@
                 break;
             }
             {
-                ti.row[threadIdx.x] = row;
+                ti.row[threadIdx.x] = row < 0 ? row : row & ~(1 << 30);
                 uint32_t have = 0;
 #pragma unroll
                 for (int k = 0; k < MAX_KVOL; ++k) {
@@ -116,7 +122,8 @@
                     }
                 }
                 const uint32_t wmask = __reduce_or_sync(0xffffffffu, have);
-                if (lane == 0) ti.mask[warp] = wmask;
+                const uint32_t wprior = __ballot_sync(0xffffffffu, row >= 0 && (row >> 30));
+                if (lane == 0) { ti.mask[warp] = wmask; ti.prior[warp] = wprior; }
                 if (threadIdx.x == 0) ti.item = x;
             }
             mbar_arrive(info_full(j & 1));
@@ -187,8 +194,27 @@
             if (x < 0) break;
             const int n_off = __popc(ti.mask[0] | ti.mask[1] | ti.mask[2] | ti.mask[3]);
             float acc[NC / 2], tot[NC / 2];
-#pragma unroll
-            for (int i = 0; i < NC / 2; ++i) tot[i] = -0.f;
+            if (p.partial_in) {
+                const int r0 = wg * 64 + (warp & 3) * 16 + (lane >> 2);
+                const float* src[2];
+#pragma unroll
+                for (int hh = 0; hh < 2; ++hh) {
+                    const int rr = r0 + 8 * hh;
+                    const bool pr = (ti.prior[rr >> 5] >> (rr & 31)) & 1u;
+                    src[hh] = pr ? p.partial_in + ((long long)((x / p.nsplit) % p.npass) * p.mout_cap + ti.row[rr]) * p.cout + (x % p.nsplit) * NC
+                                 : nullptr;
+                }
+#pragma unroll
+                for (int i = 0; i < NC / 2; i += 2) {
+                    const float* q = src[(i >> 1) & 1];
+                    const float2 t = q ? __ldcg(reinterpret_cast<const float2*>(q + 8 * (i >> 2) + 2 * (lane & 3))) : make_float2(-0.f, -0.f);
+                    tot[i] = t.x;
+                    tot[i + 1] = t.y;
+                }
+            } else {
+#pragma unroll
+                for (int i = 0; i < NC / 2; ++i) tot[i] = -0.f;
+            }
             const int n_it = n_off * p.nchunks;
             int c = 0, in_group = 0, off_idx = 0, prev_s = -1;
             for (int i = 0; i < n_it; ++i, ++it) {
@@ -226,11 +252,12 @@
             float* stage_c = reinterpret_cast<float*>(gen + (size_t)se * stage_bytes);
             {
                 const int r0 = wg * 64 + (warp & 3) * 16 + (lane >> 2);
+                const float sc = p.partial_out ? 1.f : out_scale;
 #pragma unroll
                 for (int i = 0; i < NC / 2; i += 2) {
                     const int row = r0 + 8 * ((i >> 1) & 1), col = 8 * (i >> 2) + 2 * (lane & 3);
                     *reinterpret_cast<float2*>(stage_c + row * NC + (((col >> 2) ^ (row & 7)) << 2) + (col & 3)) =
-                        make_float2(tot[i] * out_scale, tot[i + 1] * out_scale);
+                        make_float2(tot[i] * sc, tot[i + 1] * sc);
                 }
             }
             asm volatile("bar.sync 1, 256;" ::: "memory");
@@ -243,7 +270,18 @@
             const bool has_res = io.residual || io.residual_h;
             const bool gated = io.out_gated || io.out_gated_h;
             const float4 zero4 = make_float4(0.f, 0.f, 0.f, 0.f);
-            for (int e0 = 0; e0 < PER_LANE; e0 += EPI_BATCH) {
+            if (p.partial_out) {
+                float* dst = p.partial_out + (long long)((x / p.nsplit) % p.npass) * p.mout_cap * p.cout;
+                for (int e = lane; e < PER_LANE * 32; e += 32) {
+                    const int rr = cw + NUM_CONSUMER_WARPS * (e / nv);
+                    const int lcol = (e % nv) * 4;
+                    const int orow = ti.row[rr];
+                    if (orow >= 0)
+                        __stcg(reinterpret_cast<float4*>(dst + (long long)orow * p.cout + n0 + lcol),
+                               *reinterpret_cast<const float4*>(stage_c + rr * NC + (((lcol >> 2) ^ (rr & 7)) << 2)));
+                }
+            }
+            for (int e0 = 0; !p.partial_out && e0 < PER_LANE; e0 += EPI_BATCH) {
                 int orow[EPI_BATCH], col[EPI_BATCH];
                 long long gi[EPI_BATCH];
                 float4 a4[EPI_BATCH], pre4[EPI_BATCH], s4[EPI_BATCH], h4[EPI_BATCH], res4[EPI_BATCH], g4[EPI_BATCH];
@@ -413,6 +451,17 @@
     const int steps_per_offset = 3 * ((d->c1 + d->c2 + 15) / 16);
     p.group = std::max(1, tc::STEP_BUDGET / steps_per_offset);
     p.io[0] = d->io[0]; p.io[1] = d->io[d->npass > 1 ? 1 : 0];
+    p.range_mask = ~0u; p.prior_mask = 0u; p.partial_in = nullptr; p.partial_out = nullptr;
+    if (d->k1 > 0) {
+        if (d->kvol != 27 || !d->nbr || !d->row_mask || d->k0 < 0 || d->k0 >= d->k1 || d->k1 > 27 || p.group != 1 ||
+            (d->k0 > 0) != (d->partial_in != nullptr) || (d->k1 < 27) != (d->partial_out != nullptr))
+            return lb2_fail(h, LB2_ERR_ARG, "offset range: needs kvol 27, a map with row masks, c1 + c2 >= 176, 0 <= k0 < k1 <= 27, "
+                                            "partial_in iff k0 > 0 and partial_out iff k1 < 27%s", "");
+        p.range_mask = ((1u << d->k1) - 1u) & ~((1u << d->k0) - 1u);
+        p.prior_mask = (1u << d->k0) - 1u;
+        p.partial_in = d->partial_in;
+        p.partial_out = d->partial_out;
+    }
     switch (nc) {
         case 32: return tc::launch<32>(h, s, p, stages);
         case 64: return tc::launch<64>(h, s, p, stages);
diff --git a/lidiff_b200/engine.py b/lidiff_b200/engine.py
--- a/lidiff_b200/engine.py
+++ b/lidiff_b200/engine.py
@@ -2,6 +2,7 @@
 
 import math
 import os
+import re
 from collections import ChainMap
 
 import numpy as np
@@ -14,6 +15,36 @@
 GATE_NAMES = ("stage1", "stage2", "stage3", "stage4", "up1", "up2", "up3", "up4")
 GATE_LEVEL = (0, 1, 2, 3, 4, 3, 2, 1)
 BN_EPS = 1e-5
+
+OFFSET_RANGES = {2: ((0, 14), (14, 27)), 3: ((0, 9), (9, 18), (18, 27))}
+OFFSET_SPLIT_DEFAULT = {"stage4": 3, "up1": 3, "up2": 3}
+
+
+def offset_split_table(env=None):
+    env = os.environ.get("LB2_OFFSET_SPLIT", "") if env is None else env
+    table = dict(OFFSET_SPLIT_DEFAULT)
+    env = env.strip()
+    if env.isdigit():
+        return {k: int(env) for k in table}
+    for item in filter(None, env.split(",")):
+        k, _, v = item.partition("=")
+        table[k.strip()] = int(v)
+    for k, g in table.items():
+        if g != 1 and g not in OFFSET_RANGES:
+            raise ValueError(f"LB2_OFFSET_SPLIT: {k}={g} (G must be 1, 2 or 3)")
+    return table
+
+
+def split_level(name: str):
+    m = re.match(r"(stage(\d))\.[12]\.net\.[03]$", name) or re.match(r"(up(\d))\.1\.[01]\.net\.[03]$", name)
+    if m is None:
+        return None
+    n = int(m.group(2))
+    return m.group(1), (n if name.startswith("stage") else 4 - n)
+
+
+def one_offset_per_group(cin: int) -> bool:
+    return 64 // (3 * ((cin + 15) // 16)) <= 1
 
 
 class ConvLayer:
@@ -118,6 +149,8 @@
         self.pairs_of = {}
         self.pl_scratch = torch.zeros(64, **i32)
         want = [use_pairs and l in self.pair_level_set for l in range(self.pair_levels)]
+        self.split_groups = {}
+        self.range_of = {}
         self.pair_in = [torch.zeros(26 * n_cap, **i32) if w else None for w in want]
         self.pair_out = [torch.zeros(26 * n_cap, **i32) if w else None for w in want]
         self.koff = [torch.zeros(28, **i32) for _ in range(self.pair_levels)]
@@ -125,6 +158,7 @@
 
     def build(self, coords_f: torch.Tensor, n_points: int, after_levels=None, late_stream=None, late_done=None):
         h, N = self.h, self.n_cap
+        i32 = dict(dtype=torch.int32, device=coords_f.device)
         h.unique_build(coords_f, None, None, n_points, 0, self.grid[0], self.C[0], self.inv[0], self.d_n[0], self.scratch)
         for l in range(1, self.levels):
             h.unique_build(None, self.C[l - 1], self.d_n[l - 1], N, 1 << l, self.grid[l], self.C[l], self.inv[l], self.d_n[l], self.scratch)
@@ -150,6 +184,14 @@
                     to = self.tile_order_of[nbr.data_ptr()] = (torch.zeros((N + 127) // 128, dtype=torch.int32, device=nbr.device),
                                                                torch.zeros((N + 255) // 256, dtype=torch.int32, device=nbr.device))
                 h.tile_order(mask, perm, self.d_n[l_out], N, to[0], to[1], to_scratch)
+            for G in (sorted(self.split_groups.get(l_out, ())) if ks == 3 else ()):
+                ent = self.range_of.get((nbr.data_ptr(), G))
+                if ent is None:
+                    ent = self.range_of[(nbr.data_ptr(), G)] = [
+                        (k0, k1, torch.zeros(N, **i32), torch.zeros(1, **i32), torch.zeros((N + 127) // 128, **i32)) for k0, k1 in OFFSET_RANGES[G]]
+                for k0, k1, perm_r, live_r, to_r in ent:
+                    h.row_order_range(mask, self.d_n[l_out], N, k0, k1, perm_r, live_r, ro_scratch)
+                    h.tile_order_range(mask, perm_r, self.d_n[l_out] if k1 == 27 else live_r, N, k0, k1, to_r, to_scratch)
             self.map_id[nbr.data_ptr()] = slot
             self.perm_of[nbr.data_ptr()] = perm
 
@@ -257,6 +299,18 @@
         self._perm_lookup = {}
         self._tile_order_lookup = {}
         self.geom = Geometry(h, self.cap, with_up=True)
+        self.split_of = {}
+        if hasattr(h, "row_order_range") and conv_algo != _lib.ALGO_FFMA:
+            table = offset_split_table()
+            for net in (self.diff, self.refine or {}):
+                for name, lay in net.items():
+                    sl = split_level(name)
+                    if sl is None or lay.kvol != 27 or lay.Wp is None or not one_offset_per_group(lay.cin):
+                        continue
+                    G = table.get(sl[0], 1)
+                    if G > 1:
+                        self.split_of[id(lay)] = G
+                        self.geom.split_groups.setdefault(sl[1], set()).add(G)
         self._perm_lookup = self.geom.perm_of
         self._mask_lookup = self.geom.mask_of
         self._tile_order_lookup = self.geom.tile_order_of
@@ -426,18 +480,34 @@
             self.layer_log.append(dict(name=lay.name, scatter=sd is not None, map=map_ptr, d_m=d_m.data_ptr() if d_m is not None else None,
                                        cin=lay.cin, cout=lay.cout, kvol=lay.kvol, npass=npass,
                                        tc=bool(lay.Wp is not None and self.conv_algo != _lib.ALGO_FFMA)))
+        ranges = None
+        if sd is None and perm is not None and id(lay) in self.split_of:
+            ranges = self.geom.range_of.get((nbr.data_ptr(), self.split_of[id(lay)]))
         if self.conv_events is not None:
             e0, e1 = torch.cuda.Event(enable_timing=True), torch.cuda.Event(enable_timing=True)
             e0.record()
             if sd is not None:
                 self.h.spconv_scatter(sd)
-            self.h.spconv(d, self.conv_algo)
+            self._spconv(d, ranges, d_m, cap)
             e1.record()
             self.conv_events.append((e0, e1, self._conv_counter))
             self._conv_counter += 1
         else:
             if sd is not None:
                 self.h.spconv_scatter(sd)
+            self._spconv(d, ranges, d_m, cap)
+
+    def _spconv(self, d, ranges, d_m, cap):
+        if ranges is None:
+            self.h.spconv(d, self.conv_algo)
+            return
+        part = self.buf("offset_split.partial", (2, cap, 256)).data_ptr()
+        for k0, k1, perm_r, live_r, to_r in ranges:
+            d.row_perm, d.tile_order128, d.tile_order256 = perm_r.data_ptr(), to_r.data_ptr(), None
+            d.d_mout = (d_m if k1 == 27 else live_r).data_ptr()
+            d.k0, d.k1 = k0, k1
+            d.partial_in = part if k0 > 0 else None
+            d.partial_out = part if k1 < 27 else None
             self.h.spconv(d, self.conv_algo)
 
     def _res(self, L, p, geom, lvl, in1: Act, in2: Act, npass, tag, gate=None, want_plain=True, lean=False, out_f32=False):
@@ -751,7 +821,7 @@
         return list(zip(refined.split([6 * c for c in counts]), post.split(counts)))
 
 
-ENGINE_BYTES_PER_ROW = 120_000
+ENGINE_BYTES_PER_ROW = 122_000
 MAX_BATCH = 1 << 10
 
 
```

Result: faster. 30.92 (median of 6 runs) (+8.7%).
